# nttcslab-sp/torchain

Measured on AMD Instinct MI355X. Metric: sequence-frames/sec through denominator fwd-bwd, higher is better.
Workload: dtype f32

## Files before the change

### torchain_amd/csrc/chain_internal.h

```cpp
#pragma once

#include <hip/hip_runtime.h>

#include <cstdint>
#include <map>
#include <mutex>
#include <string>
#include <vector>

#include "torchain_hip.h"

namespace tc {

constexpr int kThreads = 1024;
constexpr int kWaves = kThreads / 64;
constexpr int kJvSmall = 2048 / kThreads, kPvSmall = 1024 / kThreads, kJvLarge = 4096 / kThreads, kPvLarge = 3072 / kThreads;
constexpr int kPvMid = 2048 / kThreads;
constexpr int kJvMid = 3072 / kThreads;
constexpr int kMaxRowLen = 32;
constexpr int kLdsLimitBytes = 160 * 1024;

struct ArcRec {
  float w;
  uint32_t idx;
};

constexpr uint32_t kRowFlag = 1u;
constexpr int kStreamUnroll = 16;
constexpr int kStreamUnrollTied = 8;
constexpr int kTiedMinChunks = 6;
constexpr int kMaxIndex = 1 << 14;
constexpr int kJvPlanes = 7;
constexpr int kMaxPlanePositions = 4096 * kJvPlanes;
constexpr int kJvPlanesSplit = 10;
constexpr int kMaxSplitPositions = 4096 * kJvPlanesSplit;

struct ScheduleHost {
  std::vector<ArcRec> cells;
  std::vector<uint32_t> cells6;
  std::vector<int2> wave_range;
  std::vector<int32_t> fix_begin;
  std::vector<int2> fix;
  int32_t extra_slots = 0;
  int64_t conflict_cost = 0, conflict_free_cost = 0, conflict_bound = 0;
  int64_t real_arcs = 0, padded_arcs = 0;
  int32_t rows = 0;
  std::vector<uint32_t> masks;
  int32_t mask_stride = 0;
  std::vector<int32_t> extra_first;
  int32_t nfix = 0;
  int32_t subs = 0;
  int32_t halves = 1;
};

struct ScheduleDev {
  const ArcRec *cells;
  const int2 *wave_range;
  const int32_t *fix_begin;
  const int2 *fix;
  const uint32_t *masks = nullptr;
  const int32_t *extra_first = nullptr;
  int32_t mask_stride = 0, nfix = 0;
  const void *cells_pair = nullptr;
  int32_t subs = 0;
  int32_t halves = 1;
};

constexpr int kSlabRowsPerBlock = 64;
struct SlabRow {
  int32_t row;
  int32_t n;
  int32_t f_off, s_off;
  float ws, pi;
  float K;
  float pad;
};
struct SlabListDev {
  const SlabRow *rows = nullptr;
  const int2 *head = nullptr;
  const uint32_t *rec = nullptr;
  int32_t bundles = 0;
};
struct SlabListHost {
  int W = 2, G = 16;
  std::vector<SlabRow> rows;
  std::vector<int32_t> head;
  std::vector<uint32_t> rec;
  int32_t bundles = 0;
};

struct BigDev {
  SlabListDev in, out, pdf;
  int G = 16;
  int in_blocks = 0, out_blocks = 0;
  int hb = 0;
  int tied = 0;
  const int32_t *f_off = nullptr;
};

struct DenGraphDev {
  BigDev big;
  ScheduleDev fwd, bwd;
  const float *pi;
  const uint32_t *tied_fs = nullptr;
  const float *tied_w = nullptr;
  void *blob = nullptr;
  int pair_choice = -1;
  float tune_ms[2] = {0.f, 0.f};
};

struct DenBestArc {
  int32_t src, pdf;
  float logw;
};
struct DenBestDev {
  const int32_t *in_begin = nullptr;
  const DenBestArc *arcs = nullptr;
  const float *logpi = nullptr;
  void *blob = nullptr;
};
struct DenBestParams {
  DenBestDev t;
  const float *y;
  int64_t y_stride;
  int y_bct, elem;
  int S, T, H, P, Hs;
  const int32_t *seq_frames;
  float *hist;
  int32_t *pdf_out;
  int32_t *state_out;
  double *score_out;
  int resident;
};
constexpr int kDenBestSmallLds = 1024;
inline int64_t den_best_row_floats(int H) { return ((int64_t)H + 3) & ~(int64_t)3; }
inline bool den_best_resident(int H) { return 2 * 4 * den_best_row_floats(H) + kDenBestSmallLds <= (int64_t)160 * 1024; }
inline int64_t den_best_workspace_bytes(int H, int S, int T) {
  return (((int64_t)S * (T + 1) * den_best_row_floats(H) * 4) + 255) & ~(int64_t)255;
}

struct DenLayout {
  int Hs, Ps;
  int off_a, off_acc, off_g, off_al, off_red, off_asum, total_floats;
  bool alpha_in_lds;
  int off_p2;
  int JV, PV;
  int acc_floats;
  bool planewise = false;
  bool asum_global = false;
  int src_planes = 0;
};

struct DenParams {
  ScheduleDev fwd, bwd;
  const float *pi;
  const float *y;
  int64_t y_stride;
  float *deriv;
  int64_t deriv_stride;
  float *alpha_hist;
  float *asum_g = nullptr;
  float *src_scratch = nullptr, *part_scratch = nullptr;
  double *seq_logprob;
  double *seq_y2;
  float *seq_ab;
  float *seq_gsum;
  int S, T, H, P;
  float leaky, deriv_weight, l2_scale;
  int y_vec, d_vec;
  uint32_t seq_frames_lo = 0;
  float *xent_zero = nullptr;
  int64_t xent_stride = 0;
  int x_vec = 0;
  DenLayout L;
  const uint32_t *tied_fs;
  const float *tied_w;
  int gen_owner = 0;
  uint32_t seq_frames_hi = 0;
  BigDev big;
  float *big_expy;
  int64_t big_exp_stride = 0;
  float *big_beta;
  float *big_y;
  uint32_t *big_gam = nullptr;
  float *big_small;
  int big_Sp;
  float big_sum_pi;
  long long *stamps;
  float *beta_hist = nullptr;
  float *fwd_norm = nullptr;
  float *bwd_norm = nullptr;
  float *pair_norm = nullptr;
  uint32_t *pair_sync = nullptr;
  long long *pair_stamps = nullptr;
  int pair_extra_slots = 0;
  int pair_choice = 0;
  uint32_t *mitm_sync = nullptr;
  __host__ __device__ const int32_t *seq_frames() const {
    return reinterpret_cast<const int32_t *>(((uint64_t)seq_frames_hi << 32) | seq_frames_lo);
  }
  void set_seq_frames(const int32_t *f) {
    seq_frames_lo = (uint32_t)(uintptr_t)f;
    seq_frames_hi = (uint32_t)((uint64_t)(uintptr_t)f >> 32);
  }
};

__device__ __forceinline__ int ragged_frames(const int32_t *seq_frames, int s, int T) {
  const int f = __builtin_amdgcn_readfirstlane(seq_frames[s]);
  return f < 1 ? 1 : (f > T ? T : f);
}

}

struct tc_den_graph {
  int32_t H = 0, P = 0;
  int64_t A = 0;
  std::vector<int32_t> arc_src, arc_dst, arc_pdf;
  std::vector<float> arc_prob;
  std::vector<float> initial_probs;
  tc::ScheduleHost fwd, bwd;
  bool tied = false;
  bool gen_owner = false;
  std::vector<uint32_t> tied_fs;
  std::vector<float> tied_w;
  std::vector<uint32_t> tied_fs_state;
  std::vector<float> tied_w_state;
  int32_t work_H = 0;
  std::vector<int32_t> work_src, work_dst, work_pdf, copy_first;
  std::vector<float> work_prob, work_pi;
  std::vector<int32_t> pos;
  std::vector<float> pi_pos;
  tc::DenLayout layout;
  bool layout_ok = false;
  bool big = false;
  tc::SlabListHost big_in, big_out, big_pdf;
  int big_hb = 0;
  int big_G = 16;
  std::vector<int32_t> big_f_off;
  std::vector<int32_t> tied_f, tied_s;
  float big_sum_pi = 0.f;
  std::mutex mu;
  std::map<int, tc::DenGraphDev> dev;
  std::map<int, int> preset_variant;
  std::map<int, tc::DenBestDev> best_dev;
};

namespace tc {

struct NumTables {
  std::vector<int32_t> seq_state_off, seq_arc_off, seq_uniq_off;
  std::vector<int32_t> level_begin;
  std::vector<int32_t> out_begin;
  std::vector<int32_t> in_begin;
  std::vector<int32_t> in_arc;
  std::vector<int32_t> arc_src, arc_dst, arc_uniq;
  std::vector<float> arc_logw;
  std::vector<float> final_logw;
  std::vector<int32_t> uniq_t, uniq_pdf;
  std::vector<int32_t> uniq_begin;
  std::vector<int32_t> uniq_arc;
  int32_t max_states = 0, max_arcs = 0, max_uniq = 0;
  std::vector<int32_t> frame_uniq;
  int32_t max_level_states = 0, max_level_arcs = 0, max_frame_uniq = 0;
  std::vector<int32_t> seq_level_off;
};

inline size_t num_resident_lds_bytes(int32_t max_states, int32_t max_arcs, int32_t max_uniq) {
  return (size_t)((max_states + 1) & ~1) * 16 + (size_t)((max_uniq + 3) & ~3) * 4 + (size_t)((max_arcs + 3) & ~3) * 4;
}
inline size_t num_windowed_lds_bytes(int32_t level_states, int32_t level_arcs, int32_t frame_uniq) {
  return (size_t)((level_states + 1) & ~1) * 32 + (size_t)((frame_uniq + 3) & ~3) * 4 + (size_t)((level_arcs + 3) & ~3) * 4;
}
inline bool num_windowed_fits(size_t dynamic_bytes) { return dynamic_bytes + 2048 <= (size_t)kLdsLimitBytes; }

struct E2eTables {
  std::vector<int32_t> state_off, arc_off, pdf_off, start;
  std::vector<int32_t> in_begin, out_begin;
  std::vector<uint32_t> in_key, out_key;
  std::vector<float> in_lw, out_lw;
  std::vector<int32_t> pdf_begin, pdf_arc;
  std::vector<int32_t> pdf_of;
  std::vector<float> final_lw;
  int32_t max_states = 0, max_arcs = 0, max_pdfs = 0;
  int64_t total_states = 0, total_pdfs = 0;
};

constexpr int64_t kE2eMaxScratchBytes = (int64_t)4 << 30;
struct E2eDev {
  const int32_t *state_off, *arc_off, *pdf_off, *start, *in_begin, *out_begin, *pdf_begin, *pdf_arc, *pdf_of;
  const uint32_t *in_key, *out_key;
  const float *in_lw, *out_lw, *final_lw;
  double *alpha_hist;
  int32_t max_states, max_arcs, max_pdfs;
  int32_t occ_off256;
};
static_assert(sizeof(E2eDev) == 15 * sizeof(void *) + 16, "E2eDev: NumParams' layout is part of the resident kernels' code");

struct PoolSlot {
  char *blob = nullptr, *host = nullptr;
  size_t cap = 0;
  hipEvent_t ready = nullptr, done = nullptr;
};

struct NumDev {
  const int32_t *seq_state_off, *seq_arc_off, *seq_uniq_off, *level_begin, *out_begin, *in_begin, *in_arc,
      *arc_src, *arc_dst, *arc_uniq, *uniq_t, *uniq_pdf, *uniq_begin, *uniq_arc;
  const float *arc_logw, *final_logw;
  const int32_t *frame_uniq = nullptr;
  double *alpha_hist = nullptr;
  float *stage = nullptr;
  PoolSlot *slot = nullptr;
  size_t upload_bytes = 0;
  bool uploaded = false;
  int e2e = 0;
  E2eDev e2e_tab = {};
};

struct NumParams {
  NumDev t;
  const float *y;
  int64_t y_stride;
  float *deriv;
  int64_t deriv_stride;
  float *xent;
  int64_t xent_stride;
  double *seq_logprob;
  int S, T, P;
  float weight;
  float deriv_scale = 1.f, xent_scale = 1.f;
  int staged = 0;
  const float *xent_out = nullptr;
  int64_t xent_out_stride = 0;
  double *seq_xent = nullptr;
  int xent_bct = 0, xent_out_bct = 0, y_bct = 0;
  int lds_states, lds_arcs, lds_uniq;
  int win_states, win_arcs, win_uniq;
  int elem = TC_DTYPE_F32;
  const float *xent_row_w = nullptr;
  const int32_t *seq_frames = nullptr;
  const int32_t *seq_level_off = nullptr;
  int32_t *best_pdf = nullptr;
  double *best_score = nullptr;
  const float *xent_lse = nullptr;
};

}

struct tc_supervision {
  float weight = 1.f;
  int32_t S = 0, T = 0, P = 0;
  bool e2e = false;
  tc::NumTables tab;
  tc::E2eTables e2e_tab;
  std::vector<int32_t> frames;
  int64_t total_frames = 0;
  std::vector<size_t> blob_off;
  std::mutex mu;
  std::map<int, tc::NumDev> dev;
  std::map<int, const int32_t *> frames_dev;
  std::map<int, const int32_t *> level_off_dev;
};

namespace tc {

int build_schedules(tc_den_graph *g);
void build_general(tc_den_graph *g);
bool detect_tied(tc_den_graph *g, std::vector<char> *special);
bool make_work_graph(tc_den_graph *g);
bool build_owner(tc_den_graph *g, const std::vector<char> &special, int max_row, bool count_only = false, bool general = false);
int arrange_half(const std::vector<std::vector<int64_t>> &lane_arcs, int steps, const int32_t *other,
                 const int32_t *pdf, std::vector<std::vector<int>> *pos_out);
int arrange_half_matching(const std::vector<std::vector<int64_t>> &lane_arcs, int steps, const int32_t *other,
                          std::vector<std::vector<int>> *pos_out, std::vector<std::vector<int>> *pad_bank,
                          int *lower_bound);
inline int round4(int x) { return (x + 3) & ~3; }
bool compute_layout(int H, int P, int T_hint, int extra_slots, bool tied, DenLayout *L, bool need_alpha = false);
constexpr int asum_stride(int T) { return (T + 2 + 3) & ~3; }
bool compute_layout_planes(int Npos, int P, int T_hint, int extra_slots, DenLayout *L);
int64_t layout_lds_bytes(const DenLayout &L, int T);

hipError_t allow_dynamic_lds(const void *kernel, size_t lds_bytes);
int launch_den(const DenParams &p, hipStream_t stream);
int launch_den_big(const DenParams &p, int accumulate, hipStream_t stream);
int launch_den_tied(const DenParams &p, int accumulate, hipStream_t stream);
int launch_den_general_owner(const DenParams &p, int accumulate, hipStream_t stream);
int launch_den_tied_planes(const DenParams &p, int accumulate, hipStream_t stream);
bool planes_mitm_fits(const DenParams &p);
int launch_den_tied_planes_mitm(const DenParams &p, int accumulate, hipStream_t stream);
int launch_den_tied_backward_only(const DenParams &p, hipStream_t stream);
int launch_den_tied_combine(const DenParams &p, int accumulate, int num_cus, hipStream_t stream);
bool split_bwd_fits(const DenLayout &L, int T);
constexpr int kSplitMaxSeq = 128;
int launch_den_tied_pair(const DenParams &p, int extra_slots, int accumulate, hipStream_t stream);
bool pair_fits(const DenLayout &L, int extra_slots, int T);
int tune_den_variant(tc_den_graph *g, int device);
std::string tuning_cache_key(uint64_t graph_hash, const char *device_name);
bool tuning_cache_get(const std::string &key, int *two_sequence_kernel);
void tuning_cache_put(const std::string &key, int two_sequence_kernel, float fused_ms, float two_sequence_ms);
int launch_den_tied_mitm(const DenParams &p, uint32_t *sync, int accumulate, hipStream_t stream);
bool mitm_fits(const DenLayout &L, int T);
size_t mitm_sync_bytes(int S);
int pair_norm_stride(int T);
size_t pair_sync_bytes(int S);
inline size_t pair_stamp_bytes(int T) { return ((size_t)2 * kWaves * (T + 2) * 8 * 8 + 255) & ~(size_t)255; }
int64_t big_small_floats(int hb, int P, int T, int Sp);
int launch_num(const NumParams &p, hipStream_t stream);
int launch_num_scatter(const NumParams &p, hipStream_t stream);
int launch_num_windowed(const NumParams &p, hipStream_t stream);
int launch_num_e2e(const NumParams &p, hipStream_t stream);
int launch_num_e2e_scatter(const NumParams &p, hipStream_t stream);
int launch_num_best_path(const NumParams &p, hipStream_t stream);
int launch_den_best_path(const DenBestParams &p, hipStream_t stream);
int den_best_tables(tc_den_graph *g, int device, DenBestDev *out);
inline size_t num_e2e_lds_bytes(int max_states, int max_arcs, int max_pdfs) {
  return (size_t)2 * ((max_states + 3) & ~3) * sizeof(double) + (((max_pdfs + 3) & ~3) + (size_t)max_arcs) * sizeof(float);
}
int launch_num_e2e_large(const NumParams &p, hipStream_t stream);
inline bool e2e_beyond_resident(int max_states, int max_arcs, int max_pdfs) {
  return max_states > TC_E2E_MAX_STATES || max_arcs > TC_E2E_MAX_ARCS || max_pdfs > TC_E2E_MAX_PDFS;
}
inline bool e2e_large_fits(int states, int pdfs) {
  return num_windowed_fits((size_t)16 * ((states + 3) & ~3) + (size_t)4 * ((pdfs + 3) & ~3));
}
inline size_t e2e_seq_lds_bytes(int max_states, int max_pdfs) {
  const size_t both = num_e2e_lds_bytes(max_states, 0, max_pdfs), rule = (size_t)kLdsLimitBytes - 2048;
  return both < rule ? both : rule;
}
struct SideStreams {
  hipStream_t den_side = nullptr, num_side = nullptr;
  hipEvent_t fork = nullptr, join = nullptr, num_fork = nullptr, num_join = nullptr;
  int num_cus = 0;
  std::recursive_mutex enqueue;
};
int side_streams(hipStream_t stream, SideStreams **out);
void side_streams_forget(hipStream_t stream);
int den_cus_used(const DenParams &p, int num_cus);
bool den_zeroes_xent(const DenParams &p, int num_cus);
int launch_finalize(const double *den_lp, const double *num_lp, const double *y2, const float *ab, const float *gs,
                    int S, int T, float sup_weight, float l2, int have_deriv, float *results, int32_t *fail_flag,
                    hipStream_t stream, const double *xent_lp = nullptr, double *xent_total = nullptr,
                    float *loss_out = nullptr, int64_t total_frames = 0);
int launch_finalize_per_sequence(const double *den_lp, const double *num_lp, const double *y2, const float *ab, const float *gs,
                                 int S, int T, float sup_weight, float l2, int have_deriv, float *results, int32_t *fail_flag,
                                 hipStream_t stream, const double *xent_lp, double *xent_total, float *loss_out,
                                 int64_t total_frames, const int32_t *seq_frames, int isolate, double *seq_results,
                                 int32_t *alive_frames);
int launch_zero_failed(void *out, int elem_bytes, int64_t sb, int64_t st, int64_t sc, int B, int T, int cols,
                       const int32_t *alive_frames, hipStream_t stream);
int launch_zero_padding(void *out, int elem_bytes, int64_t sb, int64_t st, int64_t sc, int B, int T, int cols,
                        const int32_t *seq_frames, hipStream_t stream);
int launch_zero_on_fail(const int32_t *fail_flag, float *a, int64_t a_stride, float *b, int64_t b_stride,
                        const float *y, int64_t y_stride, float l2_scale, int64_t rows, int cols, hipStream_t stream);
int launch_den_reduce(const double *den_lp, const float *ab, const float *gs, int S, double *logprob_out,
                      int32_t *status_out, hipStream_t stream);
int launch_sum_double(const double *in, int n, double scale, double *out, hipStream_t stream);
int launch_xent_total(const double *in, int n, const int32_t *fail_flag, double *out, hipStream_t stream);
int launch_step_loss(const float *results3, float *loss1, hipStream_t stream);
int64_t trace_workspace_bytes();
int launch_trace_mat_mat(const float *a, int64_t a_stride, const float *b, int64_t b_stride, int64_t rows, int cols,
                         double *partial, double *out, hipStream_t stream);
constexpr float kOutputLimit = 30.0f;
struct LastPass {
  float scale = 1.0f;
  const float *row_w = nullptr;
  float pen_c2 = 0.0f;
  const void *y = nullptr;
  int64_t y_stride = 0, y_st = 0;
  bool scaled = true;
};
bool layout_grid_ok(int B, int T);
int launch_to2d(int dtype, const void *in_bct, float *out, int B, int Cn, int T, int64_t stride2d, hipStream_t stream);
int launch_from2d(int dtype, const float *in, int64_t stride2d, void *out_bct, int B, int Cn, int T, const LastPass &lp,
                  hipStream_t stream);
int launch_widen_rows(int dtype, const void *in, int64_t in_stride, float *out, int64_t rows, int cols, hipStream_t stream);
int launch_round(int dtype, const float *in, void *out, int64_t n, int cols, const LastPass &lp, hipStream_t stream);
int launch_scale_rows(float *a, int64_t rows, int cols, const LastPass &lp, hipStream_t stream);
bool channel_last_strides_ok(int B, int T, int cols, int64_t sb, int64_t st);
int launch_rows_gather(int dtype, const void *x, int64_t sb, int64_t st, float *out, int64_t out_stride, int B, int T, int cols,
                       hipStream_t stream);
int launch_rows_scatter(int dtype, const float *in, int64_t in_stride, void *out, int64_t osb, int64_t ost, int B, int T,
                        int cols, const LastPass &lp, hipStream_t stream);

int launch_xent_row_stats(int dtype, const void *x, int x_bct, int64_t x_stride, int S, int T, int P, float *stats,
                          hipStream_t stream);
int launch_xent_softmax_grad(int dtype, const void *x, int x_bct, int64_t x_stride, float *g, int64_t g_stride, int S, int T,
                             int P, const float *stats, const int32_t *live_frames, hipStream_t stream);

extern thread_local int g_last_hip_error;

constexpr int kKernelGeneration = 6;
enum DebugFlag { kDbgForceGeneral = 0, kDbgForceStreamed, kDbgNoSplit, kDbgNoPdfBanks, kDbgNoBankSearch, kDbgSchedTrace, kDbgNoPhaseSplit, kDbgNoNumOverlap, kDbgNoPair, kDbgForcePair, kDbgNoTune, kDbgNoMitm, kDbgForceMitm, kDbgSlabWide, kDbgSlabNarrow, kDbgExpPerFrame, kDbgOldArrange, kDbgNoPlanes, kDbgOldGeneral, kDbgPhantomPdf0, kDbgNoPdfSearch, kDbgNoSplitSrc, kDbgPlanesMeetAt, kDbgForceNumWindowed, kDbgForceDenBestStreamed, kDbgForceNumE2eLarge, kDbgCount };
bool debug_flag(DebugFlag f);
int debug_value(DebugFlag f);

int pool_acquire(int device, size_t bytes, PoolSlot **out);
void pool_release(int device, PoolSlot *slot);
int64_t pool_counter(int which);
enum LaunchCounter { kCntDen = 0, kCntDenBackward, kCntNum, kCntNumBackward, kCntLayout, kCntDenAsumGlobal, kCntNumE2eStaged, kCntNumWindowed, kCntChannelLast, kCntRagged, kCntRaggedTwoCu, kCntBestPath, kCntDenBestPath, kCntDenBestPathStreamed, kCntXentLogSoftmax, kCntNumE2eLarge, kCntCount };
void count_launch(LaunchCounter c);
int supervision_mark_use(tc_supervision *sup, int device, hipStream_t stream);
int stage_e2e_locked(tc_supervision *sup, int device);
int supervision_from_example(const tc_example *ex, tc_supervision **out);
#define TC_HIP_CHECK(expr)                        \
  do {                                            \
    hipError_t e__ = (expr);                      \
    if (e__ != hipSuccess) {                      \
      tc::g_last_hip_error = (int)e__;            \
      return TC_ERR_HIP;                          \
    }                                             \
  } while (0)

}
```

### torchain_amd/csrc/den_graph.cpp

```cpp
#include <algorithm>
#include <atomic>
#include <array>
#include <cctype>
#include <cmath>
#include <cstdio>
#include <cstring>
#include <numeric>
#include <string>

#include "chain_internal.h"

namespace tc {

thread_local int g_last_hip_error = 0;

hipError_t allow_dynamic_lds(const void *kernel, size_t lds_bytes) {
  static std::mutex mu;
  static std::map<std::pair<const void *, int>, size_t> granted;
  int device = 0;
  hipError_t e = hipGetDevice(&device);
  if (e != hipSuccess) return e;
  std::lock_guard<std::mutex> lock(mu);
  size_t &have = granted[std::make_pair(kernel, device)];
  if (have >= lds_bytes) return hipSuccess;
  e = hipFuncSetAttribute(kernel, hipFuncAttributeMaxDynamicSharedMemorySize, (int)lds_bytes);
  if (e == hipSuccess) have = lds_bytes;
  return e;
}

static std::mutex &g_side_mu = *new std::mutex();
static std::map<std::pair<int, hipStream_t>, SideStreams> &g_side_ctx = *new std::map<std::pair<int, hipStream_t>, SideStreams>();

void side_streams_forget(hipStream_t stream) {
  int device = 0;
  if (hipGetDevice(&device) != hipSuccess) return;
  std::lock_guard<std::mutex> lock(g_side_mu);
  auto it = g_side_ctx.find(std::make_pair(device, stream));
  if (it == g_side_ctx.end()) return;
  SideStreams &c = it->second;
  for (hipStream_t x : {c.den_side, c.num_side})
    if (x) {
      (void)hipStreamSynchronize(x);
      (void)hipStreamDestroy(x);
    }
  for (hipEvent_t x : {c.fork, c.join, c.num_fork, c.num_join})
    if (x) (void)hipEventDestroy(x);
  g_side_ctx.erase(it);
}

int side_streams(hipStream_t stream, SideStreams **out) {
  std::mutex &mu = g_side_mu;
  auto &ctx = g_side_ctx;
  int device = 0;
  TC_HIP_CHECK(hipGetDevice(&device));
  std::lock_guard<std::mutex> lock(mu);
  SideStreams &c = ctx[std::make_pair(device, stream)];
  if (!c.den_side) {
    int num_cus = 0;
    TC_HIP_CHECK(hipDeviceGetAttribute(&num_cus, hipDeviceAttributeMultiprocessorCount, device));
    hipEvent_t ev[4] = {nullptr, nullptr, nullptr, nullptr};
    hipStream_t st[2] = {nullptr, nullptr};
    hipError_t e = hipSuccess;
    for (int i = 0; i < 4 && e == hipSuccess; ++i) e = hipEventCreateWithFlags(&ev[i], hipEventDisableTiming);
    for (int i = 0; i < 2 && e == hipSuccess; ++i) e = hipStreamCreateWithFlags(&st[i], hipStreamNonBlocking);
    if (e != hipSuccess) {
      for (hipEvent_t x : ev)
        if (x) (void)hipEventDestroy(x);
      for (hipStream_t x : st)
        if (x) (void)hipStreamDestroy(x);
      g_last_hip_error = (int)e;
      return TC_ERR_HIP;
    }
    c.fork = ev[0];
    c.join = ev[1];
    c.num_fork = ev[2];
    c.num_join = ev[3];
    c.num_side = st[0];
    c.den_side = st[1];
    c.num_cus = num_cus;
  }
  *out = &c;
  return TC_OK;
}

static std::atomic<int> g_debug[kDbgCount];
bool debug_flag(DebugFlag f) { return g_debug[f].load(std::memory_order_relaxed) != 0; }
int debug_value(DebugFlag f) { return g_debug[f].load(std::memory_order_relaxed); }
static std::atomic<int64_t> g_launches[kCntCount];
void count_launch(LaunchCounter c) { g_launches[c].fetch_add(1, std::memory_order_relaxed); }

struct SlabEntry {
  uint32_t d[4];
};
static uint32_t f2u(float f) {
  uint32_t u;
  std::memcpy(&u, &f, 4);
  return u;
}

static void make_slab_list(int W, int G, const std::vector<std::vector<SlabEntry>> &entries, const std::vector<SlabRow> &meta,
                           const std::vector<int32_t> &bundle_rows, SlabListHost *out) {
  const int spc = 16 / W, NG = 64 / G, CH = NG * 16;
  out->W = W;
  out->G = G;
  out->bundles = (int32_t)(bundle_rows.size() / NG);
  out->rows.assign(bundle_rows.size(), SlabRow{-1, 0, -1, -1, 0.f, 0.f, 0.f, 0.f});
  out->head.assign((size_t)out->bundles * 2, 0);
  out->rec.clear();
  size_t chunk = 0;
  for (int32_t b = 0; b < out->bundles; ++b) {
    const int32_t *br = &bundle_rows[(size_t)b * NG];
    const bool shared = NG > 1 && br[1] == -2;
    int steps = 0;
    if (shared) {
      steps = ((int)entries[br[0]].size() + NG - 1) / NG;
    } else {
      for (int q = 0; q < NG; ++q)
        if (br[q] >= 0) steps = std::max(steps, (int)entries[br[q]].size());
    }
    const int chunks = (steps + spc - 1) / spc;
    out->head[(size_t)b * 2] = (int32_t)chunk;
    out->head[(size_t)b * 2 + 1] = shared ? (int32_t)((uint32_t)steps | 0x80000000u) : steps;
    out->rec.resize((chunk + chunks) * CH, 0u);
    auto put = [&](int q, int i, const SlabEntry &e) {
      for (int c = 0; c < W; ++c) out->rec[(chunk + i / spc) * CH + q * 16 + (i % spc) * W + c] = e.d[c];
    };
    if (shared) {
      const int32_t r = br[0];
      const int n = (int)entries[r].size();
      for (int q = 0; q < NG; ++q) {
        SlabRow m = q == 0 ? meta[r] : SlabRow{-1, 0, -1, -1, 0.f, 0.f, 0.f, 0.f};
        m.n = (n - q + NG - 1) / NG;
        out->rows[(size_t)b * NG + q] = m;
      }
      for (int i = 0; i < n; ++i) put(i % NG, i / NG, entries[r][i]);
    } else {
      for (int q = 0; q < NG; ++q) {
        const int32_t r = br[q];
        if (r < 0) continue;
        SlabRow m = meta[r];
        m.n = (int32_t)entries[r].size();
        out->rows[(size_t)b * NG + q] = m;
        for (int i = 0; i < m.n; ++i) put(q, i, entries[r][i]);
      }
    }
    chunk += chunks;
  }
  out->rec.resize((chunk + 3) * CH, 0u);
}

constexpr size_t kSlabHubLen = 48;
static std::vector<int32_t> bundles_by_length(const std::vector<std::vector<SlabEntry>> &entries, int G) {
  const int NG = 64 / G;
  std::vector<int32_t> order(entries.size());
  std::iota(order.begin(), order.end(), 0);
  std::stable_sort(order.begin(), order.end(), [&](int32_t a, int32_t b) { return entries[a].size() > entries[b].size(); });
  std::vector<int32_t> out;
  size_t i = 0;
  for (; NG > 1 && i < order.size() && entries[order[i]].size() >= kSlabHubLen; ++i) {
    out.push_back(order[i]);
    for (int q = 1; q < NG; ++q) out.push_back(-2);
  }
  for (; i < order.size(); ++i) out.push_back(order[i]);
  while (out.size() % NG) out.push_back(-1);
  if (out.empty()) out.assign(NG, -1);
  return out;
}

static std::vector<int32_t> bundles_by_tile(const std::vector<std::vector<SlabEntry>> &entries, int P) {
  std::vector<int32_t> out;
  for (int p0 = 0; p0 < P; p0 += 64) {
    std::vector<int32_t> tile(64, -1);
    for (int i = 0; i < 64 && p0 + i < P; ++i) tile[i] = p0 + i;
    std::stable_sort(tile.begin(), tile.end(), [&](int32_t a, int32_t b) {
      const size_t na = a >= 0 ? entries[a].size() + 1 : 0, nb = b >= 0 ? entries[b].size() + 1 : 0;
      return na > nb;
    });
    out.insert(out.end(), tile.begin(), tile.end());
  }
  return out;
}

static void build_big(tc_den_graph *g) {
  const int H = g->H, P = g->P, G = g->big_G;
  const uint32_t rb = 4u * G;
  const int64_t A = g->A;
  std::vector<std::vector<SlabEntry>> in(H), outl(H), pdf(P);
  for (int64_t a = 0; a < A; ++a) {
    const uint32_t s = (uint32_t)g->arc_src[a] * rb, d = (uint32_t)g->arc_dst[a] * rb, pd = (uint32_t)g->arc_pdf[a] * rb;
    const uint32_t w = f2u(g->arc_prob[a]), pis = f2u(g->initial_probs[g->arc_src[a]]);
    in[g->arc_dst[a]].push_back(SlabEntry{{s, pd, w, pis}});
    outl[g->arc_src[a]].push_back(SlabEntry{{d, pd, w, f2u(1.0f)}});
    pdf[g->arc_pdf[a]].push_back(SlabEntry{{s, d, w, pis}});
  }
  std::vector<SlabRow> ms(H), mp(P);
  for (int h = 0; h < H; ++h) ms[h] = SlabRow{h, 0, -1, -1, 0.f, g->initial_probs[h], 0.f, 0.f};
  for (int i = 0; i < P; ++i) mp[i] = SlabRow{i, 0, -1, -1, 0.f, 0.f, 0.f, 0.f};
  make_slab_list(4, G, in, ms, bundles_by_length(in, G), &g->big_in);
  make_slab_list(4, G, outl, ms, bundles_by_length(outl, G), &g->big_out);
  make_slab_list(4, G, pdf, mp, bundles_by_tile(pdf, P), &g->big_pdf);
  g->big_f_off.assign(1, -1);
  float sum_pi = 0.f;
  for (int h = 0; h < H; ++h) sum_pi += g->initial_probs[h];
  g->big_sum_pi = sum_pi;
}

static void build_big_tied(tc_den_graph *g, const std::vector<char> &special) {
  const int H = g->work_H, G = g->big_G;
  const uint32_t rb = 4u * G;
  const int64_t A = (int64_t)g->work_src.size();
  std::vector<std::vector<SlabEntry>> in(H), outl(H);
  std::vector<float> K(H, 0.f);
  for (int64_t a = 0; a < A; ++a) {
    if (special[a]) continue;
    const int32_t s = g->work_src[a], d = g->work_dst[a];
    in[d].push_back(SlabEntry{{(uint32_t)s * rb, f2u(g->work_prob[a]), 0u, 0u}});
    outl[s].push_back(SlabEntry{{(uint32_t)d * rb, f2u(g->work_prob[a]), 0u, 0u}});
    K[d] += g->work_prob[a] * g->work_pi[s];
  }
  std::vector<SlabRow> mi(H), mo(H);
  g->big_f_off.assign(H, -1);
  for (int h = 0; h < H; ++h) {
    const int32_t f = g->tied_f[h] >= 0 ? g->tied_f[h] * (int32_t)rb : -1, sl = g->tied_s[h] >= 0 ? g->tied_s[h] * (int32_t)rb : -1;
    mi[h] = SlabRow{h, 0, f, sl, g->tied_w[h], g->work_pi[h], K[h], 0.f};
    mo[h] = SlabRow{h, 0, f, sl, g->tied_w[h], g->work_pi[h], 0.f, 0.f};
    g->big_f_off[h] = f;
  }
  make_slab_list(2, G, in, mi, bundles_by_length(in, G), &g->big_in);
  make_slab_list(2, G, outl, mo, bundles_by_length(outl, G), &g->big_out);
  g->big_pdf = SlabListHost();
  float sum_pi = 0.f;
  for (int h = 0; h < H; ++h) sum_pi += g->work_pi[h];
  g->big_sum_pi = sum_pi;
}

int build_schedules(tc_den_graph *g) {
  bool want_big = debug_flag(kDbgForceStreamed) || g->H > kMaxSplitPositions || g->P > kMaxIndex;
  bool split_made = false;
  std::vector<char> special;
  {
    g->work_H = g->H;
    g->work_src = g->arc_src;
    g->work_dst = g->arc_dst;
    g->work_pdf = g->arc_pdf;
    g->work_prob = g->arc_prob;
    g->work_pi = g->initial_probs;
    g->copy_first.resize(g->H + 1);
    std::iota(g->copy_first.begin(), g->copy_first.end(), 0);
    bool tied = !debug_flag(kDbgForceGeneral) && detect_tied(g, &special);
    if (!tied && !debug_flag(kDbgForceGeneral) && !debug_flag(kDbgNoSplit) && make_work_graph(g)) {
      tied = detect_tied(g, &special);
      split_made = tied;
    }
    g->tied = tied;
    if (!tied && g->H > kMaxIndex) want_big = true;
  }
  auto restore_unsplit = [&]() {
    g->work_H = g->H;
    g->work_src = g->arc_src;
    g->work_dst = g->arc_dst;
    g->work_pdf = g->arc_pdf;
    g->work_prob = g->arc_prob;
    g->work_pi = g->initial_probs;
    g->copy_first.resize(g->H + 1);
    std::iota(g->copy_first.begin(), g->copy_first.end(), 0);
    g->tied = false;
    g->gen_owner = false;
    g->tied_fs.clear();
    g->tied_w.clear();
    g->fwd = ScheduleHost();
    g->bwd = ScheduleHost();
  };
  auto general_owner = [&]() {
    if (debug_flag(kDbgOldGeneral)) return false;
    const std::vector<char> none(g->work_src.size(), 0);
    int fit_row = 0;
    int64_t best_cells = -1;
    for (int max_row = kMaxRowLen; max_row <= 8 * kMaxRowLen; max_row *= 2) {
      if (!build_owner(g, none, max_row, true, true)) continue;
      const int64_t cells = g->fwd.padded_arcs + g->bwd.padded_arcs;
      if (best_cells < 0 || cells < best_cells) {
        best_cells = cells;
        fit_row = max_row;
      }
    }
    if (!fit_row || !build_owner(g, none, fit_row, false, true)) {
      g->fwd = ScheduleHost();
      g->bwd = ScheduleHost();
      return false;
    }
    g->gen_owner = true;
    g->layout_ok = true;
    return true;
  };
  if (!want_big && g->tied) {
    int fit_row = 0;
    {
      int64_t best_cells = -1;
      for (int max_row = kMaxRowLen; max_row <= 8 * kMaxRowLen; max_row *= 2) {
        if (!build_owner(g, special, max_row, true)) continue;
        const int64_t cells = g->fwd.padded_arcs + g->bwd.padded_arcs;
        if (best_cells < 0 || cells < best_cells) {
          best_cells = cells;
          fit_row = max_row;
        }
        if (debug_flag(kDbgSchedTrace)) fprintf(stderr, "[sched] rows cut at %d: %lld cells, %d bytes of LDS\n", max_row, (long long)cells, 4 * g->layout.total_floats);
      }
      if (fit_row && !build_owner(g, special, fit_row)) {
        fit_row = 0;
        for (int max_row = kMaxRowLen; max_row <= 8 * kMaxRowLen && !fit_row; max_row *= 2)
          if (build_owner(g, special, max_row)) fit_row = max_row;
      }
    }
    if (fit_row) {
      g->layout_ok = true;
      return TC_OK;
    }
    if (split_made && g->H <= kMaxIndex) {
      std::vector<char> special_split = special;
      std::vector<int32_t> ws = g->work_src, wd = g->work_dst, wp = g->work_pdf, cf = g->copy_first, tf = g->tied_f, ts = g->tied_s;
      std::vector<float> wpr = g->work_prob, wpi = g->work_pi, tw = g->tied_w;
      std::vector<uint32_t> tfs = g->tied_fs;
      const int32_t wH = g->work_H;
      restore_unsplit();
      if (general_owner()) return TC_OK;
      build_general(g);
      g->layout_ok = compute_layout(g->H, g->P, 256, std::max(g->fwd.extra_slots, g->bwd.extra_slots), false, &g->layout);
      if (g->layout_ok) return TC_OK;
      g->work_H = wH;
      g->work_src.swap(ws);
      g->work_dst.swap(wd);
      g->work_pdf.swap(wp);
      g->work_prob.swap(wpr);
      g->work_pi.swap(wpi);
      g->copy_first.swap(cf);
      g->tied_f.swap(tf);
      g->tied_s.swap(ts);
      g->tied_w.swap(tw);
      g->tied_fs.swap(tfs);
      g->tied = true;
      special.swap(special_split);
    }
    want_big = true;
  }
  if (!want_big) {
    if (g->work_H != g->H) restore_unsplit();
    if (general_owner()) return TC_OK;
    build_general(g);
    g->layout_ok = compute_layout(g->H, g->P, 256, std::max(g->fwd.extra_slots, g->bwd.extra_slots), false, &g->layout);
    if (g->layout_ok) return TC_OK;
  }
  g->big = true;
  {
    const int64_t states = g->tied ? g->work_H : g->H;
    g->big_G = states >= 28000 ? 32 : 16;
    if (debug_flag(kDbgSlabWide)) g->big_G = 32;
    if (debug_flag(kDbgSlabNarrow)) g->big_G = 16;
  }
  g->layout_ok = false;
  g->fwd = ScheduleHost();
  g->bwd = ScheduleHost();
  if (g->tied)
    build_big_tied(g, special);
  else
    build_big(g);
  g->big_hb = (std::max(g->big_in.bundles, g->big_out.bundles) + g->big_G - 1) / g->big_G;
  return TC_OK;
}

}

using namespace tc;

extern "C" {

int tc_debug_set(const char *key, int value) {
  static const char *const names[kDbgCount] = {"force_general", "force_streamed", "no_split", "no_pdf_banks",
                                               "no_bank_search", "sched_trace", "no_phase_split", "no_num_overlap", "no_pair",
                                               "force_pair", "no_tune", "no_mitm", "force_mitm", "slab_wide", "slab_narrow", "exp_per_frame", "old_arrange", "no_planes", "old_general", "phantom_pdf0", "no_pdf_search", "no_split_source", "planes_meet_at", "force_num_windowed", "force_den_best_path_streamed", "force_num_e2e_large"};
  if (!key) return TC_ERR_INVALID_ARGUMENT;
  for (int i = 0; i < kDbgCount; ++i)
    if (!strcmp(key, names[i])) {
      g_debug[i].store(value, std::memory_order_relaxed);
      return TC_OK;
    }
  return TC_ERR_INVALID_ARGUMENT;
}

namespace {
const bool g_env_applied = [] {
  const char *env = getenv("TORCHAIN_HIP_DEBUG");
  if (!env) return false;
  std::string all(env);
  size_t pos = 0;
  while (pos <= all.size()) {
    size_t end = all.find(',', pos);
    if (end == std::string::npos) end = all.size();
    std::string item = all.substr(pos, end - pos);
    pos = end + 1;
    if (item.empty()) continue;
    int value = 1;
    const size_t eq = item.find('=');
    if (eq != std::string::npos) {
      value = atoi(item.c_str() + eq + 1);
      item.resize(eq);
    }
    if (tc_debug_set(item.c_str(), value) != TC_OK) fprintf(stderr, "libtorchain_hip: unknown switch '%s' in TORCHAIN_HIP_DEBUG\n", item.c_str());
  }
  return true;
}();
}

int64_t tc_debug_counter(const char *key) {
  if (key && !strcmp(key, "pool_device_allocs")) return pool_counter(0);
  if (key && !strcmp(key, "pool_reuses")) return pool_counter(1);
  static const char *const names[kCntCount] = {"den_launches", "den_backward_launches", "num_launches", "num_backward_launches", "layout_launches",
                                              "den_long_utterance_launches", "num_e2e_staged_launches", "num_windowed_launches", "channel_last_steps", "ragged_steps", "ragged_two_cu_launches", "best_path_launches", "den_best_path_launches", "den_best_path_streamed_launches", "xent_log_softmax_launches", "num_e2e_large_launches"};
  for (int i = 0; key && i < kCntCount; ++i)
    if (!strcmp(key, names[i])) return g_launches[i].load(std::memory_order_relaxed);
  return -1;
}

int tc_den_graph_create(tc_den_graph **out, int32_t num_states, int64_t num_arcs, const int32_t *arc_src,
                        const int32_t *arc_dst, const int32_t *arc_ilabel, const float *arc_weight,
                        const float *final_weight, int32_t start_state, int32_t num_pdfs) {
  if (!out) return TC_ERR_INVALID_ARGUMENT;
  *out = nullptr;
  if (num_states <= 0 || num_arcs < 0 || num_pdfs <= 0 || !final_weight) return TC_ERR_INVALID_ARGUMENT;
  if (num_arcs > 0 && (!arc_src || !arc_dst || !arc_ilabel || !arc_weight)) return TC_ERR_INVALID_ARGUMENT;
  if (start_state < 0 || start_state >= num_states) return TC_ERR_BAD_FST;
  if (num_arcs >= (int64_t)1 << 30) return TC_ERR_UNSUPPORTED;
  for (int64_t a = 0; a < num_arcs; ++a) {
    if (arc_src[a] < 0 || arc_src[a] >= num_states || arc_dst[a] < 0 || arc_dst[a] >= num_states)
      return TC_ERR_BAD_FST;
    if (arc_ilabel[a] < 1 || arc_ilabel[a] > num_pdfs) return TC_ERR_BAD_FST;
    if (a > 0 && arc_src[a] < arc_src[a - 1]) return TC_ERR_BAD_FST;
    if (!(arc_weight[a] == arc_weight[a])) return TC_ERR_BAD_FST;
  }
  tc_den_graph *g = new tc_den_graph();
  g->H = num_states;
  g->P = num_pdfs;
  g->A = num_arcs;
  g->arc_src.assign(arc_src, arc_src + num_arcs);
  g->arc_dst.assign(arc_dst, arc_dst + num_arcs);
  g->arc_pdf.resize(num_arcs);
  g->arc_prob.resize(num_arcs);
  for (int64_t a = 0; a < num_arcs; ++a) {
    g->arc_pdf[a] = arc_ilabel[a] - 1;
    g->arc_prob[a] = (float)std::exp(-(double)arc_weight[a]);
  }
  {
    const int H = num_states;
    std::vector<double> norm(H), cur(H, 0.0), nxt(H, 0.0), avg(H, 0.0);
    for (int s = 0; s < H; ++s) norm[s] = std::exp(-(double)final_weight[s]);
    for (int64_t a = 0; a < num_arcs; ++a) norm[arc_src[a]] += std::exp(-(double)arc_weight[a]);
    for (int s = 0; s < H; ++s)
      if (!(norm[s] > 0.0) || !std::isfinite(norm[s])) {
        delete g;
        return TC_ERR_BAD_FST;
      }
    for (int s = 0; s < H; ++s) norm[s] = 1.0 / norm[s];
    cur[start_state] = 1.0;
    for (int iter = 0; iter < 100; ++iter) {
      for (int s = 0; s < H; ++s) avg[s] += cur[s] * (1.0 / 100);
      for (int64_t a = 0; a < num_arcs; ++a) {
        int s = arc_src[a];
        nxt[arc_dst[a]] += cur[s] * norm[s] * std::exp(-(double)arc_weight[a]);
      }
      double sum = 0.0;
      for (int s = 0; s < H; ++s) sum += nxt[s];
      for (int s = 0; s < H; ++s) {
        cur[s] = nxt[s] * (1.0 / sum);
        nxt[s] = 0.0;
      }
    }
    g->initial_probs.resize(H);
    for (int s = 0; s < H; ++s) g->initial_probs[s] = (float)avg[s];
  }
  build_schedules(g);
  *out = g;
  return TC_OK;
}

}

namespace {
struct Reader {
  FILE *f;
  bool ok = true;
  template <class T>
  T get() {
    T v{};
    if (fread(&v, sizeof(T), 1, f) != 1) ok = false;
    return v;
  }
  std::string str() {
    int32_t n = get<int32_t>();
    if (!ok || n < 0 || n > (1 << 20)) {
      ok = false;
      return std::string();
    }
    std::string s((size_t)n, '\0');
    if (n && fread(&s[0], 1, (size_t)n, f) != (size_t)n) ok = false;
    return s;
  }
  void skip_symbol_table() {
    int32_t magic = get<int32_t>();
    if (magic != 2125658996) {
      ok = false;
      return;
    }
    str();
    get<int64_t>();
    int64_t size = get<int64_t>();
    for (int64_t i = 0; ok && i < size; ++i) {
      str();
      get<int64_t>();
    }
  }
};
}

extern "C" {

int tc_den_graph_read(tc_den_graph **out, const char *rxfilename, int32_t num_pdfs) {
  if (!out || !rxfilename) return TC_ERR_INVALID_ARGUMENT;
  *out = nullptr;
  std::string name(rxfilename);
  while (!name.empty() && isspace((unsigned char)name.back())) name.pop_back();
  const bool is_pipe = !name.empty() && name.back() == '|';
  if (is_pipe) name.pop_back();
  FILE *f = is_pipe ? popen(name.c_str(), "r") : fopen(name.c_str(), "rb");
  if (!f) return TC_ERR_IO;
  Reader r{f};
  int rc = TC_OK;
  std::vector<int32_t> src, dst, il;
  std::vector<float> w, fin;
  int64_t start = 0, nstates = 0;
  try {
  do {
    if (r.get<int32_t>() != 2125659606) { rc = TC_ERR_IO; break; }
    std::string fsttype = r.str(), arctype = r.str();
    int32_t version = r.get<int32_t>(), flags = r.get<int32_t>();
    r.get<uint64_t>();
    start = r.get<int64_t>();
    nstates = r.get<int64_t>();
    int64_t narcs = r.get<int64_t>();
    if (!r.ok || fsttype != "vector" || arctype != "standard" || version < 2 || (flags & 4)  ||
        nstates <= 0 || nstates > (1 << 24)) {
      rc = TC_ERR_IO;
      break;
    }
    if (flags & 1) r.skip_symbol_table();
    if (flags & 2) r.skip_symbol_table();
    if (narcs > 0 && narcs <= (1 << 24)) { src.reserve(narcs); dst.reserve(narcs); il.reserve(narcs); w.reserve(narcs); }
    fin.resize(nstates);
    for (int64_t s = 0; r.ok && s < nstates; ++s) {
      fin[s] = r.get<float>();
      int64_t n = r.get<int64_t>();
      if (!r.ok || n < 0 || n > (1 << 28)) { r.ok = false; break; }
      for (int64_t i = 0; r.ok && i < n; ++i) {
        int32_t ilabel = r.get<int32_t>();
        r.get<int32_t>();
        float weight = r.get<float>();
        int32_t next = r.get<int32_t>();
        src.push_back((int32_t)s);
        dst.push_back(next);
        il.push_back(ilabel);
        w.push_back(weight);
      }
    }
    if (!r.ok) rc = TC_ERR_IO;
  } while (0);
  } catch (...) {
    rc = TC_ERR_IO;
  }
  if (is_pipe) {
    if (pclose(f) != 0 && rc == TC_OK) rc = TC_ERR_IO;
  } else {
    fclose(f);
  }
  if (rc != TC_OK) return rc;
  return tc_den_graph_create(out, (int32_t)nstates, (int64_t)src.size(), src.data(), dst.data(), il.data(), w.data(),
                             fin.data(), (int32_t)start, num_pdfs);
}

void tc_den_graph_free(tc_den_graph *g) {
  if (!g) return;
  for (auto &kv : g->dev) {
    if (kv.second.blob) {
      int cur = 0;
      if (hipGetDevice(&cur) == hipSuccess) {
        (void)hipSetDevice(kv.first);
        (void)hipFree(kv.second.blob);
        (void)hipSetDevice(cur);
      }
    }
  }
  for (auto &kv : g->best_dev) {
    int cur = 0;
    if (kv.second.blob && hipGetDevice(&cur) == hipSuccess) {
      (void)hipSetDevice(kv.first);
      (void)hipFree(kv.second.blob);
      (void)hipSetDevice(cur);
    }
  }
  delete g;
}

int32_t tc_den_graph_num_states(const tc_den_graph *g) { return g ? g->H : 0; }
int64_t tc_den_graph_num_arcs(const tc_den_graph *g) { return g ? g->A : 0; }
int32_t tc_den_graph_num_pdfs(const tc_den_graph *g) { return g ? g->P : 0; }

int tc_den_graph_initial_probs(const tc_den_graph *g, float *out_host) {
  if (!g || !out_host) return TC_ERR_INVALID_ARGUMENT;
  memcpy(out_host, g->initial_probs.data(), sizeof(float) * (size_t)g->H);
  return TC_OK;
}

int tc_den_graph_stats(const tc_den_graph *g, int64_t *o) {
  if (!g || !o) return TC_ERR_INVALID_ARGUMENT;
  o[0] = g->fwd.padded_arcs;
  o[1] = g->bwd.padded_arcs;
  o[2] = g->layout_ok ? layout_lds_bytes(g->layout, 150) : -1;
  o[3] = kThreads;
  o[4] = g->fwd.rows;
  o[5] = g->bwd.rows;
  o[6] = g->fwd.conflict_free_cost ? 1000 * g->fwd.conflict_cost / g->fwd.conflict_free_cost : 0;
  o[7] = g->bwd.conflict_free_cost ? 1000 * g->bwd.conflict_cost / g->bwd.conflict_free_cost : 0;
  o[8] = g->big ? 2 : (g->tied ? 1 : 0);
  return TC_OK;
}

int tc_den_graph_debug_walk(const tc_den_graph *g, int direction, const float *gather, const float *pdf_factor,
                            float *out) {
  if (!g || !gather || !pdf_factor || !out || direction < 0 || direction > 1) return TC_ERR_INVALID_ARGUMENT;
  const int H = g->H;
  auto slab_sums = [&](const SlabListHost &L, auto term, std::vector<float> *sums) {
    const int spc = 16 / L.W, NG = 64 / L.G, CH = NG * 16;
    for (int32_t b = 0; b < L.bundles; ++b) {
      const bool shared = L.head[(size_t)b * 2 + 1] < 0;
      float gsum[4] = {0.f, 0.f, 0.f, 0.f};
      for (int q = 0; q < NG; ++q) {
        const SlabRow &r = L.rows[(size_t)b * NG + q];
        if (r.row < 0 && !shared) continue;
        float sum = 0.f;
        for (int i = 0; i < r.n; ++i) sum += term(&L.rec[((size_t)L.head[(size_t)b * 2] + i / spc) * CH + q * 16 + (i % spc) * L.W]);
        if (shared)
          gsum[q] = sum;
        else
          (*sums)[r.row] = sum;
      }
      if (shared) (*sums)[L.rows[(size_t)b * NG].row] = NG == 4 ? (gsum[0] + gsum[1]) + (gsum[2] + gsum[3]) : gsum[0] + gsum[1];
    }
  };
  auto u2f = [](uint32_t u) {
    float f;
    std::memcpy(&f, &u, 4);
    return f;
  };
  if (g->big && g->tied) {
    const SlabListHost &L = direction == 0 ? g->big_in : g->big_out;
    auto pf = [&](int pdf) { return pdf >= 0 ? pdf_factor[pdf] : 0.f; };
    std::vector<float> val(g->work_H, 0.f), sums(g->work_H, 0.f);
    for (int h = 0; h < H; ++h)
      for (int c = g->copy_first[h]; c < g->copy_first[h + 1]; ++c)
        val[c] = direction == 0 ? (c == g->copy_first[h] ? gather[h] : 0.f) : gather[h] * pf(g->tied_f[c]);
    slab_sums(L, [&](const uint32_t *e) { return u2f(e[1]) * val[e[0] / (4 * L.G)]; }, &sums);
    for (int h = 0; h < H; ++h) {
      float total = 0.f;
      for (int c = g->copy_first[h]; c < g->copy_first[h + 1]; ++c) {
        const float own = direction == 0 ? (c == g->copy_first[h] ? gather[h] : 0.f) : gather[h];
        const float self = pf(g->tied_s[c]) * g->tied_w[c] * own;
        const float v = direction == 0 ? pf(g->tied_f[c]) * sums[c] + self : sums[c] + self;
        if (direction == 1) {
          total = v;
          break;
        }
        total += v;
      }
      out[h] = total;
    }
    return TC_OK;
  }
  if (g->big) {
    std::vector<float> sums(H, 0.f);
    slab_sums(direction == 0 ? g->big_in : g->big_out,
              [&](const uint32_t *e) { return u2f(e[2]) * gather[e[0] / (4 * g->big_G)] * pdf_factor[e[1] / (4 * g->big_G)]; }, &sums);
    for (int h = 0; h < H; ++h) out[h] = sums[h];
    return TC_OK;
  }
  if (!g->layout_ok) return TC_ERR_UNSUPPORTED;
  const ScheduleHost &sc = direction == 0 ? g->fwd : g->bwd;
  const int Hs = g->layout.Hs;
  std::vector<float> acc((size_t)std::max(g->layout.acc_floats, Hs + 4 + sc.extra_slots) + 64, 0.f);
  if (g->gen_owner) {
    const int K = Hs / kThreads;
    std::vector<float> src_pos((size_t)Hs + 4, 0.f);
    for (int h = 0; h < H; ++h) src_pos[g->pos[h]] = gather[h];
    for (int w = 0; w < kWaves; ++w) {
      const int first = sc.wave_range[w].x, n = sc.wave_range[w].y;
      for (int l = 0; l < 64; ++l) {
        const int tid = 64 * w + l;
        int k = 0;
        float a = 0.f;
        auto slot = [&]() { return k < K ? 4 * (tid + kThreads * (k >> 2)) + (k & 3) : Hs + 4 + 64 * (sc.extra_first[w] + (k - K)) + l; };
        for (int i = 0; i < n; ++i) {
          const size_t c = (size_t)first + i, chunk = c / 8, q = c % 8;
          const uint32_t *base = &sc.cells6[chunk * 4 * 64 * 4];
          const uint32_t x = base[((q / 4) * 64 + l) * 4 + (q % 4)], idx = base[((2 + q / 4) * 64 + l) * 4 + (q % 4)];
          float wgt;
          memcpy(&wgt, &x, 4);
          a += wgt * src_pos[(idx & 0xffffu) >> 2] * pdf_factor[idx >> 18];
          const uint32_t m = sc.masks[(size_t)w * sc.mask_stride + (i / 2) / 8];
          const int bit = (i / 2) % 8;
          if ((m >> ((i & 1) ? bit : 8 + bit)) & 1u) {
            acc[slot()] = a;
            ++k;
            a = 0.f;
          }
        }
      }
    }
    for (size_t t = 0; t + 1 < sc.fix_begin.size(); ++t)
      for (int e = sc.fix_begin[t]; e < sc.fix_begin[t + 1]; ++e) acc[sc.fix[e].x] += acc[sc.fix[e].y];
    for (int h = 0; h < H; ++h) out[h] = acc[g->pos[h]];
    return TC_OK;
  }
  if (g->tied) {
    const int K = Hs / kThreads;
    const bool pw = g->layout.planewise;
    const int subs = pw ? sc.subs : 1, halves = pw ? sc.halves : 1, subs_all = subs * halves;
    const int half_pos = halves == 2 ? 4096 * ((Hs / 4096 + 1) / 2) : 0;
    std::vector<float> total(acc.size(), 0.f);
    std::vector<float> src_pos((size_t)Hs + 4, 0.f);
    for (int h = 0; h < H; ++h)
      for (int c = g->copy_first[h]; c < g->copy_first[h + 1]; ++c) {
        const uint32_t fs = g->tied_fs[g->pos[c]];
        src_pos[g->pos[c]] = direction == 0 ? (c == g->copy_first[h] ? gather[h] : 0.f)
                                            : gather[h] * pdf_factor[(fs & 0xffffu) >> 2];
      }
    for (int hv = 0; hv < halves; ++hv) {
    std::fill(acc.begin(), acc.end(), 0.f);
    const int pos_base = hv ? half_pos : 0;
    for (int w = 0; w < kWaves; ++w)
     for (int sub = 0; sub < subs; ++sub) {
      const int first = sc.wave_range[(size_t)w * subs_all + hv * subs + sub].x;
      const int rel = pw ? first - sc.wave_range[(size_t)w * subs_all].x : 0;
      const int n = sc.wave_range[(size_t)w * subs_all + hv * subs + sub].y - rel;
      for (int l = 0; l < 64; ++l) {
        const int tid = 64 * w + l;
        int k = !pw ? 0 : sub == 0 ? K : 4 * (sub - 1);
        float ax = 0.f, ay = 0.f;
        auto slot = [&]() {
          return k < K ? 4 * (tid + kThreads * (k >> 2)) + (k & 3) : Hs + 4 + 64 * (sc.extra_first[w] + (k - K)) + l;
        };
        auto cell = [&](int i, float *wgt, int *position) {
          const size_t c = (size_t)first + i, chunk = c / 8, q = c % 8;
          const uint32_t *base = &sc.cells6[chunk * 3 * 64 * 4];
          uint32_t x = base[((q / 4) * 64 + l) * 4 + (q % 4)];
          memcpy(wgt, &x, 4);
          const uint32_t o = base[(2 * 64 + l) * 4 + q / 2];
          *position = pos_base + (int)(((q & 1) ? o >> 16 : o & 0xffffu) >> (pw ? 0 : 2));
        };
        for (int i = 0; i < n; i += 2) {
          float w0, w1;
          int p0, p1;
          cell(i, &w0, &p0);
          cell(i + 1, &w1, &p1);
          uint32_t m = pw ? 0u : sc.masks[((size_t)w * subs + sub) * sc.mask_stride + (i / 2) / 8];
          int bit = (i / 2) % 8;
          if (pw) {
            const int cell = rel + i, chunk = cell / 8;
            const uint32_t byte = (sc.masks[(size_t)w * sc.mask_stride + chunk / 4] >> (8 * (chunk % 4))) & 0xffu;
            m = (((byte >> (cell % 8)) & 1u) << 8) | ((byte >> (cell % 8 + 1)) & 1u);
            bit = 0;
          }
          if ((m >> (8 + bit)) & 1u) {
            acc[slot()] = (ax + w0 * src_pos[p0]) + ay;
            ++k;
            ax = 0.f;
            ay = w1 * src_pos[p1];
          } else {
            ax += w0 * src_pos[p0];
            ay += w1 * src_pos[p1];
          }
          if ((m >> bit) & 1u) {
            acc[slot()] = ax + ay;
            ++k;
            ax = ay = 0.f;
          }
        }
      }
    }
    const size_t lists = (sc.fix_begin.size() - 1) / (size_t)halves;
    for (size_t t = hv * lists; t < (hv + 1) * lists; ++t)
      for (int e = sc.fix_begin[t]; e < sc.fix_begin[t + 1]; ++e) {
        const size_t tl = t - hv * lists;
        if (pw && ((sc.fix[e].x >> 2) % kThreads != (int)(tl / (K / 4)) || sc.fix[e].x / (4 * kThreads) != (int)(tl % (K / 4))))
          return TC_ERR_UNSUPPORTED;
        acc[sc.fix[e].x] += acc[sc.fix[e].y];
      }
    for (int p = 0; p < Hs; ++p) total[p] += acc[p];
    }
    acc.swap(total);
    for (int h = 0; h < H; ++h) {
      float sum = 0.f;
      for (int c = g->copy_first[h]; c < g->copy_first[h + 1]; ++c) {
        const int p = g->pos[c];
        const uint32_t fs = g->tied_fs[p];
        const float self = pdf_factor[fs >> 18] * g->tied_w[p] * (direction == 0 && c != g->copy_first[h] ? 0.f : gather[h]);
        const float v = direction == 0 ? pdf_factor[(fs & 0xffffu) >> 2] * acc[p] + self : acc[p] + self;
        if (direction == 1) {
          sum = v;
          break;
        }
        sum += v;
      }
      out[h] = sum;
    }
    return TC_OK;
  }
  for (int w = 0; w < kWaves; ++w) {
    const int first = sc.wave_range[w].x, n = sc.wave_range[w].y;
    for (int l = 0; l < 64; ++l) {
      int cur = Hs;
      float a = 0.f;
      for (int i = 0; i < n; ++i) {
        const size_t c = (size_t)first + i;
        const ArcRec &r = sc.cells[((c >> 1) * 64 + l) * 2 + (c & 1)];
        if (r.idx & kRowFlag) {
          acc[cur] = a;
          uint32_t x;
          memcpy(&x, &r.w, 4);
          cur = (int)(x & 0xffffu);
          a = 0.f;
        } else {
          a += r.w * gather[std::min<uint32_t>(r.idx >> 18, (uint32_t)H - 1)] * pdf_factor[(r.idx >> 2) & 0x3fffu];
        }
      }
    }
  }
  for (int t = 0; t < kThreads; ++t)
    for (int e = sc.fix_begin[t]; e < sc.fix_begin[t + 1]; ++e) acc[sc.fix[e].x] += acc[sc.fix[e].y];
  for (int h = 0; h < H; ++h) out[h] = acc[h];
  return TC_OK;
}

static int upload_den_graph(tc_den_graph *g, int device);

int tc_den_graph_prepare(tc_den_graph *g, int device) {
  if (!g) return TC_ERR_INVALID_ARGUMENT;
  const int rc = upload_den_graph(g, device);
  if (rc != TC_OK) return rc;
  return tune_den_variant(g, device);
}

static int upload_den_graph(tc_den_graph *g, int device) {
  std::lock_guard<std::mutex> lock(g->mu);
  if (g->dev.count(device)) return TC_OK;
  int prev = 0;
  TC_HIP_CHECK(hipGetDevice(&prev));
  TC_HIP_CHECK(hipSetDevice(device));
  const int Hs = (g->H + 3) & ~3;
  auto align = [](size_t x) { return (x + 255) & ~(size_t)255; };
  struct Part { const void *src; size_t bytes; size_t off; };
  if (g->big) {
    const std::vector<float> &pi_src = g->tied ? g->work_pi : g->initial_probs;
    std::vector<float> pi_pad(pi_src.size() + 8, 0.f);
    std::copy(pi_src.begin(), pi_src.end(), pi_pad.begin());
    const std::vector<int32_t> none_i(1, -1);
    const std::vector<float> none_f(1, 0.f);
    const bool tb = g->tied;
    const SlabListHost *lists[3] = {&g->big_in, &g->big_out, &g->big_pdf};
    const std::vector<SlabRow> no_rows(4, SlabRow{-1, 0, -1, -1, 0.f, 0.f, 0.f, 0.f});
    const std::vector<int32_t> no_head(2, 0);
    const std::vector<uint32_t> no_rec(256, 0u);
    Part parts[11];
    for (int l = 0; l < 3; ++l) {
      const bool have = lists[l]->bundles > 0;
      parts[3 * l] = Part{have ? (const void *)lists[l]->rows.data() : no_rows.data(), (have ? lists[l]->rows.size() : 4) * sizeof(SlabRow), 0};
      parts[3 * l + 1] = Part{have ? (const void *)lists[l]->head.data() : no_head.data(), (have ? lists[l]->head.size() : 2) * 4, 0};
      parts[3 * l + 2] = Part{have ? (const void *)lists[l]->rec.data() : no_rec.data(), (have ? lists[l]->rec.size() : 256) * 4, 0};
    }
    parts[9] = Part{pi_pad.data(), pi_pad.size() * 4, 0};
    parts[10] = Part{g->big_f_off.data(), g->big_f_off.size() * 4, 0};
    size_t total = 0;
    for (auto &p : parts) {
      p.off = total;
      total += align(p.bytes);
    }
    char *blob = nullptr;
    hipError_t e = hipMalloc((void **)&blob, total);
    if (e == hipSuccess)
      for (auto &p : parts) {
        e = hipMemcpy(blob + p.off, p.src, p.bytes, hipMemcpyHostToDevice);
        if (e != hipSuccess) break;
      }
    (void)hipSetDevice(prev);
    if (e != hipSuccess) {
      g_last_hip_error = (int)e;
      return TC_ERR_HIP;
    }
    DenGraphDev d;
    d.blob = blob;
    SlabListDev *dl[3] = {&d.big.in, &d.big.out, &d.big.pdf};
    for (int l = 0; l < 3; ++l) {
      dl[l]->rows = (const SlabRow *)(blob + parts[3 * l].off);
      dl[l]->head = (const int2 *)(blob + parts[3 * l + 1].off);
      dl[l]->rec = (const uint32_t *)(blob + parts[3 * l + 2].off);
      dl[l]->bundles = lists[l]->bundles;
    }
    d.pi = (const float *)(blob + parts[9].off);
    d.big.tied = tb ? 1 : 0;
    d.big.G = g->big_G;
    d.big.in_blocks = (g->big_in.bundles + g->big_G - 1) / g->big_G;
    d.big.out_blocks = (g->big_out.bundles + g->big_G - 1) / g->big_G;
    d.big.hb = g->big_hb;
    d.big.f_off = (const int32_t *)(blob + parts[10].off);
    g->dev[device] = d;
    return TC_OK;
  }
  std::vector<float> pi_pad(Hs + 4, 0.f);
  std::copy(g->initial_probs.begin(), g->initial_probs.end(), pi_pad.begin());
  if (g->tied || g->gen_owner) pi_pad = g->pi_pos;
  const std::vector<uint32_t> no_mask(1, 0u);
  const std::vector<int32_t> no_extra(kWaves, 0);
  std::vector<uint32_t> pair_cells[2];
  const bool want_pair = g->tied && g->layout.Hs <= 8192 && !g->fwd.cells6.empty();
  if (want_pair)
    for (int dir = 0; dir < 2; ++dir) {
      const std::vector<uint32_t> &src = dir == 0 ? g->fwd.cells6 : g->bwd.cells6;
      pair_cells[dir] = src;
      for (size_t chunk = 0; chunk + 1 <= src.size() / (3 * 64 * 4); ++chunk)
        for (size_t i = 0; i < 64 * 4; ++i) {
          uint32_t &x = pair_cells[dir][chunk * 3 * 64 * 4 + 2 * 64 * 4 + i];
          x = ((x & 0xffffu) << 1) | ((x >> 16) << 17);
        }
    }
  const std::vector<uint32_t> no_pair(4, 0u);
  Part parts[] = {
      {g->fwd.cells6.empty() ? (const void *)g->fwd.cells.data() : (const void *)g->fwd.cells6.data(),
       g->fwd.cells6.empty() ? g->fwd.cells.size() * sizeof(ArcRec) : g->fwd.cells6.size() * 4, 0},
      {g->fwd.wave_range.data(), g->fwd.wave_range.size() * sizeof(int2), 0},
      {g->bwd.cells6.empty() ? (const void *)g->bwd.cells.data() : (const void *)g->bwd.cells6.data(),
       g->bwd.cells6.empty() ? g->bwd.cells.size() * sizeof(ArcRec) : g->bwd.cells6.size() * 4, 0},
      {g->bwd.wave_range.data(), g->bwd.wave_range.size() * sizeof(int2), 0},
      {pi_pad.data(), pi_pad.size() * 4, 0},
      {g->fwd.fix_begin.data(), g->fwd.fix_begin.size() * 4, 0},
      {g->fwd.fix.data(), g->fwd.fix.size() * sizeof(int2), 0},
      {g->bwd.fix_begin.data(), g->bwd.fix_begin.size() * 4, 0},
      {g->bwd.fix.data(), g->bwd.fix.size() * sizeof(int2), 0},
      {g->tied_fs.data(), g->tied_fs.size() * 4, 0},
      {g->tied_w.data(), g->tied_w.size() * 4, 0},
      {g->fwd.masks.empty() ? no_mask.data() : g->fwd.masks.data(), std::max<size_t>(1, g->fwd.masks.size()) * 4, 0},
      {g->bwd.masks.empty() ? no_mask.data() : g->bwd.masks.data(), std::max<size_t>(1, g->bwd.masks.size()) * 4, 0},
      {g->fwd.extra_first.empty() ? no_extra.data() : g->fwd.extra_first.data(), kWaves * 4, 0},
      {g->bwd.extra_first.empty() ? no_extra.data() : g->bwd.extra_first.data(), kWaves * 4, 0},
      {want_pair ? pair_cells[0].data() : no_pair.data(), (want_pair ? pair_cells[0].size() : no_pair.size()) * 4, 0},
      {want_pair ? pair_cells[1].data() : no_pair.data(), (want_pair ? pair_cells[1].size() : no_pair.size()) * 4, 0},
  };
  size_t total = 0;
  for (auto &p : parts) {
    p.off = total;
    total += align(p.bytes);
  }
  char *blob = nullptr;
  hipError_t e = hipMalloc((void **)&blob, total);
  if (e == hipSuccess) {
    for (auto &p : parts) {
      e = hipMemcpy(blob + p.off, p.src, p.bytes, hipMemcpyHostToDevice);
      if (e != hipSuccess) break;
    }
  }
  (void)hipSetDevice(prev);
  if (e != hipSuccess) {
    g_last_hip_error = (int)e;
    return TC_ERR_HIP;
  }
  DenGraphDev d;
  d.blob = blob;
  d.fwd = ScheduleDev{(const ArcRec *)(blob + parts[0].off), (const int2 *)(blob + parts[1].off),
                      (const int32_t *)(blob + parts[5].off), (const int2 *)(blob + parts[6].off),
                      (const uint32_t *)(blob + parts[11].off), (const int32_t *)(blob + parts[13].off),
                      g->fwd.mask_stride, g->fwd.nfix};
  d.bwd = ScheduleDev{(const ArcRec *)(blob + parts[2].off), (const int2 *)(blob + parts[3].off),
                      (const int32_t *)(blob + parts[7].off), (const int2 *)(blob + parts[8].off),
                      (const uint32_t *)(blob + parts[12].off), (const int32_t *)(blob + parts[14].off),
                      g->bwd.mask_stride, g->bwd.nfix};
  d.fwd.subs = g->fwd.subs;
  d.bwd.subs = g->bwd.subs;
  d.fwd.halves = g->fwd.halves;
  d.bwd.halves = g->bwd.halves;
  d.pi = (const float *)(blob + parts[4].off);
  if (g->tied) {
    d.tied_fs = (const uint32_t *)(blob + parts[9].off);
    d.tied_w = (const float *)(blob + parts[10].off);
  }
  if (want_pair) {
    d.fwd.cells_pair = blob + parts[15].off;
    d.bwd.cells_pair = blob + parts[16].off;
  }
  g->dev[device] = d;
  return TC_OK;
}

}

int tc::den_best_tables(tc_den_graph *g, int device, DenBestDev *out) {
  std::lock_guard<std::mutex> lock(g->mu);
  auto it = g->best_dev.find(device);
  if (it != g->best_dev.end()) {
    *out = it->second;
    return TC_OK;
  }
  const int H = g->H;
  const int64_t A = g->A;
  std::vector<int32_t> in_begin(H + 1, 0);
  for (int64_t a = 0; a < A; ++a) ++in_begin[g->arc_dst[a] + 1];
  for (int h = 0; h < H; ++h) in_begin[h + 1] += in_begin[h];
  std::vector<DenBestArc> arcs((size_t)std::max<int64_t>(A, 1), DenBestArc{0, 0, -INFINITY});
  {
    std::vector<int32_t> fill(in_begin.begin(), in_begin.end() - 1);
    for (int64_t a = 0; a < A; ++a)
      arcs[fill[g->arc_dst[a]]++] = DenBestArc{g->arc_src[a], g->arc_pdf[a], (float)std::log((double)g->arc_prob[a])};
  }
  std::vector<float> logpi(H);
  for (int h = 0; h < H; ++h) logpi[h] = g->initial_probs[h] > 0.f ? (float)std::log((double)g->initial_probs[h]) : -INFINITY;
  auto align = [](size_t x) { return (x + 255) & ~(size_t)255; };
  const size_t off_arcs = align(in_begin.size() * 4), off_pi = off_arcs + align(arcs.size() * sizeof(DenBestArc));
  const size_t total = off_pi + align(logpi.size() * 4);
  int prev = 0;
  TC_HIP_CHECK(hipGetDevice(&prev));
  TC_HIP_CHECK(hipSetDevice(device));
  char *blob = nullptr;
  hipError_t e = hipMalloc((void **)&blob, total);
  if (e == hipSuccess) e = hipMemcpy(blob, in_begin.data(), in_begin.size() * 4, hipMemcpyHostToDevice);
  if (e == hipSuccess) e = hipMemcpy(blob + off_arcs, arcs.data(), arcs.size() * sizeof(DenBestArc), hipMemcpyHostToDevice);
  if (e == hipSuccess) e = hipMemcpy(blob + off_pi, logpi.data(), logpi.size() * 4, hipMemcpyHostToDevice);
  (void)hipSetDevice(prev);
  if (e != hipSuccess) {
    if (blob) (void)hipFree(blob);
    g_last_hip_error = (int)e;
    return TC_ERR_HIP;
  }
  DenBestDev d;
  d.in_begin = (const int32_t *)blob;
  d.arcs = (const DenBestArc *)(blob + off_arcs);
  d.logpi = (const float *)(blob + off_pi);
  d.blob = blob;
  g->best_dev[device] = d;
  *out = d;
  return TC_OK;
}

extern "C" {

const char *tc_strerror(int code) {
  switch (code) {
    case TC_OK: return "ok";
    case TC_ERR_INVALID_ARGUMENT: return "invalid argument";
    case TC_ERR_BAD_FST: return "malformed FST";
    case TC_ERR_UNSUPPORTED: return "problem size not supported by the on-chip layout";
    case TC_ERR_WORKSPACE: return "workspace missing or too small";
    case TC_ERR_HIP: return "HIP runtime error";
    case TC_ERR_IO: return "cannot read OpenFst vector/standard file";
    case TC_ERR_NOT_SEPARABLE: return "merged supervision FST does not factor per sequence";
    default: return "unknown error";
  }
}

int tc_version(void) { return 100; }
int tc_last_hip_error(void) { return tc::g_last_hip_error; }

}
```

### torchain_amd/csrc/den_tied_device.h

```cpp
#pragma once

#include "den_device.h"

namespace tc {

namespace {

typedef float f4 __attribute__((ext_vector_type(4)));
typedef uint32_t u4 __attribute__((ext_vector_type(4)));
typedef __attribute__((address_space(3))) float lds_f;
typedef __attribute__((address_space(3))) uint32_t lds_u;
typedef __attribute__((address_space(3))) f4 lds_f4;
typedef __attribute__((address_space(3))) u4 lds_u4;

__device__ __forceinline__ float ldsf(uint32_t a) { return *reinterpret_cast<lds_f *>(a); }
__device__ __forceinline__ void ldsf_st(uint32_t a, float v) { *reinterpret_cast<lds_f *>(a) = v; }
__device__ __forceinline__ f4 lds4(uint32_t a) { return *reinterpret_cast<lds_f4 *>(a); }
__device__ __forceinline__ void lds4_st(uint32_t a, f4 v) { *reinterpret_cast<lds_f4 *>(a) = v; }
__device__ __forceinline__ void lds4_st_at(uint32_t base, uint32_t off, f4 v) {
  asm volatile("ds_write_b128 %0, %1 offset:%2" : : "v"(base), "v"(v), "i"(off) : "memory");
}
__device__ __forceinline__ u4 lds4u(uint32_t a) { return *reinterpret_cast<lds_u4 *>(a); }
__device__ __forceinline__ void lds_add_u32(uint32_t a, uint32_t v) {
  __hip_atomic_fetch_add(reinterpret_cast<lds_u *>(a), v, __ATOMIC_RELAXED, __HIP_MEMORY_SCOPE_WORKGROUP);
}

typedef __amdgpu_buffer_rsrc_t rsrc_t;
__device__ __forceinline__ rsrc_t make_rsrc(const void *ubase, uint32_t bytes) {
  return __builtin_amdgcn_make_buffer_rsrc(const_cast<void *>(ubase), 0, (int)bytes, 0x00020000);
}
__device__ __forceinline__ u4 bld4u(rsrc_t r, uint32_t voff, uint32_t soff) {
  return __builtin_amdgcn_raw_buffer_load_b128(r, (int)voff, (int)soff, 0);
}
__device__ __forceinline__ f4 bld4(rsrc_t r, uint32_t voff, uint32_t soff) {
  const u4 v = bld4u(r, voff, soff);
  return f4{__uint_as_float(v.x), __uint_as_float(v.y), __uint_as_float(v.z), __uint_as_float(v.w)};
}
template <int AUX>
__device__ __forceinline__ f4 bld4_aux(rsrc_t r, uint32_t voff, uint32_t soff) {
  const u4 v = __builtin_amdgcn_raw_buffer_load_b128(r, (int)voff, (int)soff, AUX);
  return f4{__uint_as_float(v.x), __uint_as_float(v.y), __uint_as_float(v.z), __uint_as_float(v.w)};
}
__device__ __forceinline__ void bst4(rsrc_t r, uint32_t voff, f4 v) {
#ifndef TC_STORE_AUX
#define TC_STORE_AUX 2
#endif
  __builtin_amdgcn_raw_buffer_store_b128(u4{__float_as_uint(v.x), __float_as_uint(v.y), __float_as_uint(v.z), __float_as_uint(v.w)},
                                         r, (int)voff, 0, TC_STORE_AUX);
}

template <int AUX>
__device__ __forceinline__ void bst4_aux(rsrc_t r, uint32_t voff, f4 v) {
  __builtin_amdgcn_raw_buffer_store_b128(u4{__float_as_uint(v.x), __float_as_uint(v.y), __float_as_uint(v.z), __float_as_uint(v.w)},
                                         r, (int)voff, 0, AUX);
}

__device__ __forceinline__ void dma4_to_lds(rsrc_t r, uint32_t voff, uint32_t lds_wave) {
  uint32_t keep;
  asm volatile("s_mov_b32 %0, m0\n\ts_mov_b32 m0, %3\n\ts_nop 4\n\tbuffer_load_dwordx4 %1, %2, 0 offen lds\n\ts_mov_b32 m0, %0"
               : "=&s"(keep)
               : "v"(voff), "s"(r), "s"(lds_wave)
               : "memory");
}
template <int N>
__device__ __forceinline__ void dma_wait() {
  static_assert(N >= 0 && N < 64, "vmcnt is a 6-bit count");
  asm volatile("s_waitcnt vmcnt(%0)" : : "n"(N) : "memory");
}
__device__ __forceinline__ void lds_wait_all() { asm volatile("s_waitcnt lgkmcnt(0)" : : : "memory"); }

__device__ __forceinline__ f4 mk4(float x) { return f4{x, x, x, x}; }
__device__ __forceinline__ float hsum(f4 v) { return (v.x + v.y) + (v.z + v.w); }
__device__ __forceinline__ float exp_med3(float x) { return __expf(__builtin_amdgcn_fmed3f(x, -30.0f, 30.0f)); }
__device__ __forceinline__ f4 exp4(f4 y) { return f4{exp_med3(y.x), exp_med3(y.y), exp_med3(y.z), exp_med3(y.w)}; }

__device__ __forceinline__ f4 row_ld(rsrc_t r, uint32_t voff, int vec) {
  if (vec) return bld4(r, voff, 0);
  return f4{__uint_as_float(__builtin_amdgcn_raw_buffer_load_b32(r, (int)voff, 0, 0)),
            __uint_as_float(__builtin_amdgcn_raw_buffer_load_b32(r, (int)voff, 4, 0)),
            __uint_as_float(__builtin_amdgcn_raw_buffer_load_b32(r, (int)voff, 8, 0)),
            __uint_as_float(__builtin_amdgcn_raw_buffer_load_b32(r, (int)voff, 12, 0))};
}
__device__ __forceinline__ void row_st(rsrc_t r, uint32_t voff, int vec, f4 v) {
  if (vec) {
    bst4(r, voff, v);
  } else {
    __builtin_amdgcn_raw_buffer_store_b32(__float_as_uint(v.x), r, (int)voff, 0, 0);
    __builtin_amdgcn_raw_buffer_store_b32(__float_as_uint(v.y), r, (int)voff, 4, 0);
    __builtin_amdgcn_raw_buffer_store_b32(__float_as_uint(v.z), r, (int)voff, 8, 0);
    __builtin_amdgcn_raw_buffer_store_b32(__float_as_uint(v.w), r, (int)voff, 12, 0);
  }
}

__device__ __forceinline__ float block_sum_a(float v, uint32_t red, int wave, uint32_t lane) {
  v = wave_sum(v);
  if (lane == 0) ldsf_st(red + 4u * (uint32_t)wave, v);
  __syncthreads();
  static_assert(kWaves == 16, "one DPP row holds the wave totals");
  float t = ldsf(red + 4u * (lane & 15u));
  t = dpp_add<0xB1>(t);
  t = dpp_add<0x4E>(t);
  t = dpp_add<0x124>(t);
  t = dpp_add<0x128>(t);
  return t;
}

__device__ __forceinline__ void gamma_add_a(uint32_t addr, float v) {
  int32_t q;
  asm("v_cvt_rpi_i32_f32 %0, %1" : "=v"(q) : "v"(v));
  lds_add_u32(addr, (uint32_t)q);
}

struct Chunk6 {
  u4 wa, wb, oc;
};

__device__ __forceinline__ void load_chunk(Chunk6 &q, rsrc_t stream, uint32_t lane16, int chunk) {
  const uint32_t so = (uint32_t)chunk * (3 * 64 * 16);
  q.wa = bld4u(stream, lane16, so);
  q.wb = bld4u(stream, lane16, so + 1024);
  q.oc = bld4u(stream, lane16, so + 2048);
}

__device__ __forceinline__ uint32_t lo16(uint32_t x) {
  uint32_t r;
  asm volatile("v_and_b32 %0, 0xffff, %1" : "=v"(r) : "v"(x));
  return r;
}
__device__ __forceinline__ uint32_t hi16(uint32_t x) {
  uint32_t r;
  asm volatile("v_lshrrev_b32 %0, 16, %1" : "=v"(r) : "v"(x));
  return r;
}

__device__ __forceinline__ uint32_t lo16w(uint32_t x) {
  uint32_t r;
  const uint32_t two = 2u;
  asm volatile("v_lshlrev_b32_sdwa %0, %1, %2 dst_sel:DWORD dst_unused:UNUSED_PAD src0_sel:DWORD src1_sel:WORD_0" : "=v"(r) : "s"(two), "v"(x));
  return r;
}
__device__ __forceinline__ uint32_t hi16w(uint32_t x) {
  uint32_t r;
  const uint32_t two = 2u;
  asm volatile("v_lshlrev_b32_sdwa %0, %1, %2 dst_sel:DWORD dst_unused:UNUSED_PAD src0_sel:DWORD src1_sel:WORD_1" : "=v"(r) : "s"(two), "v"(x));
  return r;
}

struct RowCommit {
  uint32_t row;
  uint32_t sec_row;
  int left;
  __device__ __forceinline__ void commit(float v) {
    asm volatile("s_mov_b32 m0, %1\n\ts_nop 0\n\tds_write_addtid_b32 %0" : : "v"(v), "s"(row) : "memory", "m0");
    --left;
    row = left == 0 ? sec_row : row + 256u;
  }
};

template <uint32_t SRC, int HALF>
__device__ __forceinline__ void do_chunk(const Chunk6 &q, uint32_t m, float &acc, RowCommit &rc) {
  uint32_t o[8];
  o[0] = lo16(q.oc.x);
  o[1] = hi16(q.oc.x);
  o[2] = lo16(q.oc.y);
  o[3] = hi16(q.oc.y);
  o[4] = lo16(q.oc.z);
  o[5] = hi16(q.oc.z);
  o[6] = lo16(q.oc.w);
  o[7] = hi16(q.oc.w);
  float a[8];
#pragma unroll
  for (int i = 0; i < 8; ++i) {
#ifdef TC_ABL_NOGATHER
    a[i] = __uint_as_float(o[i]);
#else
    a[i] = ldsf(SRC + o[i]);
#endif
  }
  const uint32_t w[8] = {q.wa.x, q.wa.y, q.wa.z, q.wa.w, q.wb.x, q.wb.y, q.wb.z, q.wb.w};
#pragma unroll
  for (int i = 0; i < 8; ++i) {
    acc = fmaf(a[i], __uint_as_float(w[i]), acc);
    const int bit = (i & 1) ? 4 * HALF + i / 2 : 8 + 4 * HALF + i / 2;
    if (__builtin_expect((m >> bit) & 1u, 0)) {
      rc.commit(acc);
      acc = 0.f;
    }
  }
}

__device__ __forceinline__ uint32_t wave_masks(const ScheduleDev &sc, int wave, uint32_t lane) {
  const uint32_t i = lane < (uint32_t)sc.mask_stride ? lane : (uint32_t)sc.mask_stride - 1u;
  return sc.masks[(size_t)wave * sc.mask_stride + i];
}

constexpr int kWalkEnd = -1000;

template <uint32_t SRC, int RES, class AfterChunk>
__device__ __forceinline__ void walk(const Chunk6 (&res)[RES > 0 ? RES : 1], Chunk6 &qa, rsrc_t sbase,
                                     uint32_t lane16, int nchunks, uint32_t vmask, RowCommit rc,
                                     AfterChunk after_chunk TC_WALK_ARG) {
  static_assert(RES % 2 == 0, "a mask word covers two chunks");
  auto mk = [&](int i) { return (uint32_t)__builtin_amdgcn_readlane((int)vmask, i); };
  float acc = 0.f;
#ifdef TC_PHASE_STAMPS
  wst[2] = clock64();
#endif
#pragma unroll
  for (int i = 0; i < RES / 2; ++i) {
    const uint32_t m = mk(i);
    do_chunk<SRC, 0>(res[2 * i], m, acc, rc);
    after_chunk(2 * i);
    do_chunk<SRC, 1>(res[2 * i + 1], m, acc, rc);
    after_chunk(2 * i + 1);
  }
#ifdef TC_PHASE_STAMPS
  {
    __builtin_amdgcn_s_waitcnt(0xC07F);
    const long long now = clock64();
    wst[0] += now - wst[2];
    wst[2] = now;
  }
#endif
  Chunk6 qb;
  int c = RES;
  for (; c + 2 < nchunks; c += 2) {
    const uint32_t m = mk(c >> 1);
    load_chunk(qb, sbase, lane16, c + 1);
    do_chunk<SRC, 0>(qa, m, acc, rc);
    load_chunk(qa, sbase, lane16, c + 2);
    do_chunk<SRC, 1>(qb, m, acc, rc);
    if (RES == 0) after_chunk(-1 - (c >> 1));
  }
  if (c + 1 < nchunks) {
    const uint32_t m = mk(c >> 1);
    load_chunk(qb, sbase, lane16, c + 1);
    do_chunk<SRC, 0>(qa, m, acc, rc);
    do_chunk<SRC, 1>(qb, m, acc, rc);
  } else if (c < nchunks) {
    do_chunk<SRC, 0>(qa, mk(c >> 1), acc, rc);
  }
  if (RES == 0) after_chunk(kWalkEnd);
#ifdef TC_PHASE_STAMPS
  __builtin_amdgcn_s_waitcnt(0xC07F);
  wst[1] += clock64() - wst[2];
#endif
}

template <uint32_t SRC>
__device__ __forceinline__ void chunk_pw(const Chunk6 &q, uint32_t m8, float &acc, RowCommit &rc) {
  uint32_t o[8];
  o[0] = lo16w(q.oc.x);
  o[1] = hi16w(q.oc.x);
  o[2] = lo16w(q.oc.y);
  o[3] = hi16w(q.oc.y);
  o[4] = lo16w(q.oc.z);
  o[5] = hi16w(q.oc.z);
  o[6] = lo16w(q.oc.w);
  o[7] = hi16w(q.oc.w);
  float a[8];
#pragma unroll
  for (int i = 0; i < 8; ++i) a[i] = ldsf(SRC + o[i]);
  const uint32_t w[8] = {q.wa.x, q.wa.y, q.wa.z, q.wa.w, q.wb.x, q.wb.y, q.wb.z, q.wb.w};
#pragma unroll
  for (int i = 0; i < 8; ++i) {
    acc = fmaf(a[i], __uint_as_float(w[i]), acc);
    if (__builtin_expect((m8 >> i) & 1u, 0)) {
      rc.commit(acc);
      acc = 0.f;
    }
  }
}

__device__ __forceinline__ void age_prio_on(int wave) {
  if (wave >= 12)
    __builtin_amdgcn_s_setprio(3);
  else if (wave >= 8)
    __builtin_amdgcn_s_setprio(2);
  else if (wave >= 4)
    __builtin_amdgcn_s_setprio(1);
}

__device__ __forceinline__ float tied_alpha(uint32_t pb, uint32_t fs, float ws, float F, float a_self) {
  return fmaf(ldsf(pb + (fs & 0xffffu)), F, ldsf(pb + (fs >> 16)) * (ws * a_self));
}

__device__ __forceinline__ f4 own_rows(uint32_t vrow, int j) {
  return f4{ldsf(vrow + 256u * (4 * j)), ldsf(vrow + 256u * (4 * j + 1)), ldsf(vrow + 256u * (4 * j + 2)),
            ldsf(vrow + 256u * (4 * j + 3))};
}

__device__ __forceinline__ void fold_row(int2 f, uint32_t vrow, uint32_t aACC, int Hs, int K) {
  const int k = 4 * (f.x / (4 * kThreads)) + (f.x & 3);
  const uint32_t dst = vrow + 256u * (uint32_t)k;
  const uint32_t src = aACC + 256u * (uint32_t)(K * kWaves) + 4u * (uint32_t)(f.y - Hs - 4);
  ldsf_st(dst, ldsf(dst) + ldsf(src));
}

__device__ __forceinline__ void fold_row_pw(int2 f, uint32_t vrow, uint32_t aACC, int Hs) {
  const uint32_t dst = vrow + 256u * (uint32_t)(f.x & 3);
  const uint32_t src = aACC + 256u * (uint32_t)(4 * kWaves) + 4u * (uint32_t)(f.y - Hs - 4);
  ldsf_st(dst, ldsf(dst) + ldsf(src));
}

constexpr uint32_t kPlane = 16u * kThreads;

struct AsumRow {
  uint32_t lds;
  float *g;
  __device__ __forceinline__ AsumRow(const DenParams &p, int s)
      : lds(4u * (uint32_t)p.L.off_asum), g(p.L.asum_global ? p.asum_g + (int64_t)s * asum_stride(p.T) : nullptr) {}
  __device__ __forceinline__ void st(int t, float v) const {
    if (g)
      g[t] = v;
    else
      ldsf_st(lds + 4u * (uint32_t)t, v);
  }
  __device__ __forceinline__ float ld(int t) const {
    if (g) return __uint_as_float(__builtin_amdgcn_raw_buffer_load_b32(make_rsrc(g + t, 4u), 0, 0, 0));
    return ldsf(lds + 4u * (uint32_t)t);
  }
};

}

#define TC_TIED_DISPATCH(CALL)                            \
  if (JV == kJvSmall && PV == kPvSmall) return CALL(kJvSmall, kPvSmall); \
  if (JV == kJvSmall && PV == kPvMid) return CALL(kJvSmall, kPvMid);     \
  if (JV == kJvSmall && PV == kPvLarge) return CALL(kJvSmall, kPvLarge); \
  if (JV == kJvMid && PV == kPvSmall) return CALL(kJvMid, kPvSmall);     \
  if (JV == kJvMid && PV == kPvMid) return CALL(kJvMid, kPvMid);         \
  if (JV == kJvMid && PV == kPvLarge) return CALL(kJvMid, kPvLarge);     \
  if (JV == kJvLarge && PV == kPvSmall) return CALL(kJvLarge, kPvSmall); \
  if (JV == kJvLarge && PV == kPvMid) return CALL(kJvLarge, kPvMid);     \
  if (JV == kJvLarge && PV == kPvLarge) return CALL(kJvLarge, kPvLarge);

}
```

### torchain_amd/csrc/den_tied_frames.h

```cpp
#pragma once

#include <type_traits>

#include "den_tied_device.h"

namespace tc {

__device__ __forceinline__ void block_sum2(float &v1, float &v2, uint32_t red, int wave, uint32_t lane) {
  v1 = wave_sum(v1);
  v2 = wave_sum(v2);
  if (lane == 0) {
    ldsf_st(red + 4u * (uint32_t)wave, v1);
    ldsf_st(red + 4u * (uint32_t)(kWaves + wave), v2);
  }
  __syncthreads();
  float t1 = ldsf(red + 4u * (lane & 15u)), t2 = ldsf(red + 4u * (kWaves + (lane & 15u)));
  t1 = dpp_add<0xB1>(t1);
  t2 = dpp_add<0xB1>(t2);
  t1 = dpp_add<0x4E>(t1);
  t2 = dpp_add<0x4E>(t2);
  t1 = dpp_add<0x124>(t1);
  t2 = dpp_add<0x124>(t2);
  v1 = dpp_add<0x128>(t1);
  v2 = dpp_add<0x128>(t2);
}

__device__ __forceinline__ float vload_f32(const float *ptr) {
  return __uint_as_float(__builtin_amdgcn_raw_buffer_load_b32(make_rsrc(ptr, 4u), 0, 0, 0));
}

template <bool GAMMA>
__device__ __forceinline__ float tied_fwd_state(uint32_t pb, uint32_t aGM, float inv_prev, uint32_t fsx, float wsx, float Fx, float alx,
                                                float bx, float gs, float &dpart) {
  const float pf = ldsf(pb + (fsx & 0xffffu)), ps = ldsf(pb + (fsx >> 16));
  const float sp = ps * (wsx * alx);
  const float a = fmaf(pf, Fx, sp) * inv_prev;
  if constexpr (GAMMA) {
    const float g = gs * bx, spn = sp * inv_prev;
    gamma_add_a(aGM + (fsx >> 16), g * spn);
    gamma_add_a(aGM + (fsx & 0xffffu), g * fmaxf(a - spn, 0.f));
    dpart = fmaf(a, bx, dpart);
  }
  return a;
}
template <bool PURE>
__device__ __forceinline__ float tied_bwd_state(uint32_t pb, uint32_t aGM, uint32_t fsx, float wsx, float bo, float alx, float aupx,
                                                float cpx, float ax, float inv_as, float asum_up) {
  const float ps_ws = ldsf(pb + (fsx >> 16)) * wsx;
  if constexpr (!PURE) {
    const float selfpart = ps_ws * alx * inv_as;
    const float bos = kGammaScale * bo;
    gamma_add_a(aGM + (fsx >> 16), bos * selfpart);
#ifndef TC_ABL_NOFADD
    gamma_add_a(aGM + (fsx & 0xffffu), bos * fmaxf((aupx - cpx * asum_up) - selfpart, 0.f));
#endif
  }
  return fmaf(ps_ws, bo, ax);
}

template <int JV, int PV, bool ALPHA_LDS, bool ACCUM, int RESF, int RESB, bool MITM>
struct TiedSeq {
  const DenParams &p;
  const uint32_t tid, lane;
  const int wave, s;
  const int H, P, S, T, Hs, Ps;
  const int planes, K;
  const uint32_t own16, lane16;
  static constexpr uint32_t kPB = 0u;
  static constexpr uint32_t kA0 = PV * 16u * kThreads;
  const uint32_t aACC;
  const uint32_t vrow;
  const uint32_t aGM;
  const uint32_t aAL;
  const uint32_t aRed, aAsum;
  const uint32_t tab_bytes, row_bytes;
  const rsrc_t r_pi, r_fs, r_ws;
  const float leaky;
  const int64_t hist_step;
  float *const hist;
  float *const fn;
  float *const bn;
  float *const bhist;
  const int M;

  int fnch, store_slot, bnch, bstore_slot;
  uint32_t fsec, bsec;
  uint32_t aFS, aWS;
  bool tabs_lds;
  uint32_t pb_cur, pb_next;
  rsrc_t fbase, bbase;
  float asum, inv_prev, bsum;
  float chat;
  float part, y2, part_tot;
  int ffx0, ffx1, bfx0, bfx1;
  uint32_t fmask, bmask;
  Chunk6 fres[RESF > 0 ? RESF : 1];
  Chunk6 bres[RESB > 0 ? RESB : 1];
  f4 v4[JV];
  f4 bt[JV];
  f4 areg[JV];
  f4 ycur[PV], ynext[PV];
  f4 bown[JV];
#ifdef TC_PHASE_STAMPS
  long long st_prev, st_acc[8];
#endif

  __device__ __forceinline__ TiedSeq(const DenParams &pp, int seq, int meet, int frames = 0)
      : p(pp), tid(threadIdx.x), lane(threadIdx.x & 63u), wave(__builtin_amdgcn_readfirstlane(threadIdx.x >> 6)), s(seq),
        H(pp.H), P(pp.P), S(pp.S), T(frames > 0 ? frames : pp.T), Hs(pp.L.Hs), Ps(pp.L.Ps), planes(pp.L.Hs / (4 * kThreads)), K(pp.L.Hs / kThreads),
        own16(16u * threadIdx.x), lane16(16u * (threadIdx.x & 63u)), aACC(4u * (uint32_t)pp.L.off_acc),
        vrow(4u * (uint32_t)pp.L.off_acc + 256u * (uint32_t)((pp.L.Hs / kThreads) * __builtin_amdgcn_readfirstlane(threadIdx.x >> 6)) +
             4u * (threadIdx.x & 63u)),
        aGM(4u * (uint32_t)pp.L.off_g), aAL(4u * (uint32_t)pp.L.off_al), aRed(4u * (uint32_t)pp.L.off_red),
        aAsum(4u * (uint32_t)pp.L.off_asum), tab_bytes(4u * (uint32_t)(pp.L.Hs + 4)), row_bytes(4u * (uint32_t)pp.P),
        r_pi(make_rsrc(pp.pi, 4u * (uint32_t)(pp.L.Hs + 4))), r_fs(make_rsrc(pp.tied_fs, 4u * (uint32_t)(pp.L.Hs + 4))),
        r_ws(make_rsrc(pp.tied_w, 4u * (uint32_t)(pp.L.Hs + 4))), leaky(pp.leaky), hist_step((int64_t)pp.S * pp.L.Hs),
        hist(pp.alpha_hist + (int64_t)seq * pp.L.Hs), fn(MITM ? pp.fwd_norm + (int64_t)seq * (pp.T + 2) : nullptr),
        bn(MITM ? pp.bwd_norm + (int64_t)seq * (pp.T + 1) : nullptr), bhist(MITM ? pp.beta_hist + (int64_t)seq * pp.L.Hs : nullptr),
        M(meet) {}

  __device__ __forceinline__ bool plane_on(int j) const { return j < planes; }

  __device__ __forceinline__ void stamps_reset() {
#ifdef TC_PHASE_STAMPS
    st_prev = clock64();
    for (int i = 0; i < 8; ++i) st_acc[i] = 0;
#endif
  }
  __device__ __forceinline__ void stamps_flush(int base) {
#ifdef TC_PHASE_STAMPS
    TC_STAMP(0)
    if (!MITM && blockIdx.x == 0 && lane == 0)
      for (int i = 0; i < 8; ++i) p.stamps[base + wave * 8 + i] = st_acc[i];
#endif
  }

  __device__ __forceinline__ void xent_zero_row(int t) {
    if (p.xent_zero) {
      const rsrc_t xrow = make_rsrc(p.xent_zero + ((int64_t)t * S + s) * p.xent_stride, row_bytes);
#pragma unroll
      for (int v = 0; v < PV; ++v)
        if (4 * ((int)tid + kThreads * v) < Ps) row_st(xrow, own16 + v * kPlane, p.x_vec, mk4(0.f));
    }
  }

  template <bool GAMMA>
  __device__ __forceinline__ float fwd_state(uint32_t fsx, float wsx, float Fx, float alx, float bx, float gs, float &dpart) {
    return tied_fwd_state<GAMMA>(kPB, aGM, inv_prev, fsx, wsx, Fx, alx, bx, gs, dpart);
  }
  template <bool PURE>
  __device__ __forceinline__ float bwd_state(uint32_t pb, uint32_t fsx, float wsx, float bo, float alx, float aupx, float cpx, float ax,
                                             float inv_as, float asum_up) {
    return tied_bwd_state<PURE>(pb, aGM, fsx, wsx, bo, alx, aupx, cpx, ax, inv_as, asum_up);
  }

  __device__ __forceinline__ void forward_begin() {
    f4 pi4[JV];
    part = 0.f;
#pragma unroll
    for (int j = 0; j < JV; ++j) {
      pi4[j] = plane_on(j) ? bld4(r_pi, own16, j * kPlane) : mk4(0.f);
      part += hsum(pi4[j]);
    }
    asum = block_sum_a(part, aRed, wave, lane);
#pragma unroll
    for (int j = 0; j < JV; ++j)
      if (plane_on(j)) {
        const f4 a = pi4[j] + (leaky * pi4[j]) * asum;
        lds4_st(kA0 + own16 + j * kPlane, a);
        bst4(make_rsrc(hist, 4u * Hs), own16 + j * kPlane, a);
      }
    y2 = 0.f;
    {
      const rsrc_t yrow = make_rsrc(p.y + (int64_t)s * p.y_stride, row_bytes);
#pragma unroll
      for (int v = 0; v < PV; ++v) {
        const int i0 = 4 * ((int)tid + kThreads * v);
        if (i0 < Ps) {
          const f4 yv = row_ld(yrow, own16 + v * kPlane, p.y_vec);
          y2 += hsum(yv * yv);
          lds4_st(kPB + 4u * i0, exp4(yv));
        }
      }
    }
    if (tid == 0) {
      ldsf_st(aAsum, asum);
      if (MITM) fn[0] = asum;
    }
    inv_prev = __builtin_amdgcn_rcpf(asum);

    {
    const int2 frange = p.fwd.wave_range[wave];
#ifdef TC_ABL_NOSTREAM
    fnch = RESF;
#else
    fnch = __builtin_amdgcn_readfirstlane(frange.y) / kChunk;
#endif
    fbase = make_rsrc(reinterpret_cast<const char *>(p.fwd.cells) +
                          (int64_t)(__builtin_amdgcn_readfirstlane(frange.x) / kChunk) * (3 * 64 * 16),
                      (uint32_t)(fnch + 2) * (3 * 64 * 16));
    fmask = wave_masks(p.fwd, wave, lane);
    ffx0 = p.fwd.nfix ? p.fwd.fix_begin[tid] : 0;
    ffx1 = p.fwd.nfix ? p.fwd.fix_begin[tid + 1] : 0;
    fsec = aACC + 256u * (uint32_t)(K * kWaves + p.fwd.extra_first[wave]);
#pragma unroll
    for (int i = 0; i < RESF; ++i) load_chunk(fres[i], fbase, lane16, i);
    }
    tabs_lds = (p.L.off_red - p.L.off_g) >= 2 * Hs;
    aFS = aGM;
    aWS = aGM + 4u * (uint32_t)Hs;
    if (tabs_lds) {
#pragma unroll
      for (int j = 0; j < JV; ++j)
        if (plane_on(j)) {
          *reinterpret_cast<lds_u4 *>(aFS + own16 + j * kPlane) = bld4u(r_fs, own16, j * kPlane);
          lds4_st(aWS + own16 + j * kPlane, bld4(r_ws, own16, j * kPlane));
        }
    }
    store_slot = RESF >= 4 ? wave >> 2 : RESF >= 2 ? wave >> 3 : 0;
#pragma unroll
    for (int j = 0; j < JV; ++j) v4[j] = bt[j] = mk4(0.f);
    chat = 0.f;
    part_tot = 0.f;
    stamps_reset();
  }

  static constexpr bool kHistFromPass = !MITM;

  template <bool GAMMA>
  __device__ __forceinline__ void forward_frame(int t) {
#ifdef TC_PHASE_STAMPS
    long long *const wst = st_acc + 5;
#endif
    TC_STAMP(0)
    Chunk6 q0;
    load_chunk(q0, fbase, lane16, RESF);
    __syncthreads();
    TC_STAMP(1)
    f4 yreg[PV];
    if (t < T) {
      const rsrc_t yrow = make_rsrc(p.y + ((int64_t)t * S + s) * p.y_stride, row_bytes);
#pragma unroll
      for (int v = 0; v < PV; ++v) yreg[v] = row_ld(yrow, own16 + v * kPlane, p.y_vec);
    }
    float n_t = 1.f;
    if (GAMMA && t < T) n_t = vload_f32(bn + t);
    age_prio_on(wave);
    bool stored = false;
    const RowCommit frc{aACC + 256u * (uint32_t)(K * wave), fsec, K};
    walk<kA0, RESF>(fres, q0, fbase, lane16, fnch, fmask, frc, [&](int i) {
      if (!kHistFromPass && !GAMMA && t > 1 && !stored && (RESF > 0 ? i == store_slot : (i == kWalkEnd || i == -1 - (wave >> 2)))) {
        stored = true;
        const rsrc_t hist_prev = make_rsrc(hist + (int64_t)(t - 1) * hist_step, 4u * Hs);
#ifndef TC_ABL_NOHIST
#pragma unroll
        for (int j = 0; j < JV; ++j)
          if (plane_on(j)) bst4(hist_prev, own16 + j * kPlane, lds4(kA0 + own16 + j * kPlane));
#endif
      }
    } TC_WALK_PASS);
    __builtin_amdgcn_s_setprio(0);
    TC_STAMP(2)
    for (int e = ffx0; e < ffx1; ++e) fold_row(p.fwd.fix[e], vrow, aACC, Hs, K);
    TC_STAMP(3)
    part = 0.f;
    float dpart = 0.f;
    u4 fs[JV];
    f4 ws[JV], cpi[JV];
#pragma unroll
    for (int j = 0; j < JV; ++j)
      if (plane_on(j)) {
        fs[j] = tabs_lds ? lds4u(aFS + own16 + j * kPlane) : bld4u(r_fs, own16, j * kPlane);
        ws[j] = tabs_lds ? lds4(aWS + own16 + j * kPlane) : bld4(r_ws, own16, j * kPlane);
        cpi[j] = bld4(r_pi, own16, j * kPlane);
      }
    const float gs = kGammaScale * chat;
    const rsrc_t hist_prev = make_rsrc(hist + (int64_t)(t - 1) * hist_step, t > 1 ? 4u * Hs : 0u);
#pragma unroll
    for (int j = 0; j < JV; ++j) {
      v4[j] = mk4(0.f);
      if (plane_on(j)) {
        const f4 F = own_rows(vrow, j);
        const f4 al = lds4(kA0 + own16 + j * kPlane);
#ifndef TC_ABL_NOHIST
        if (kHistFromPass && !GAMMA) bst4(hist_prev, own16 + j * kPlane, al);
#endif
        v4[j] = f4{fwd_state<GAMMA>(fs[j].x, ws[j].x, F.x, al.x, bt[j].x, gs, dpart), fwd_state<GAMMA>(fs[j].y, ws[j].y, F.y, al.y, bt[j].y, gs, dpart),
                   fwd_state<GAMMA>(fs[j].z, ws[j].z, F.z, al.z, bt[j].z, gs, dpart), fwd_state<GAMMA>(fs[j].w, ws[j].w, F.w, al.w, bt[j].w, gs, dpart)};
        part += hsum(v4[j]);
      }
    }
    f4 yp[PV];
    if (GAMMA) {
      const rsrc_t yprev = make_rsrc(p.y + ((int64_t)(t - 1) * S + s) * p.y_stride, row_bytes);
#pragma unroll
      for (int v = 0; v < PV; ++v) yp[v] = row_ld(yprev, own16 + v * kPlane, p.y_vec);
      const rsrc_t brow = make_rsrc(bhist + (int64_t)(t + 1 <= T ? t + 1 : T) * hist_step, 4u * Hs);
#pragma unroll
      for (int j = 0; j < JV; ++j) bt[j] = bld4(brow, own16, j * kPlane);
      block_sum2(part, dpart, aRed, wave, lane);
      asum = part;
    } else {
      asum = block_sum_a(part, aRed, wave, lane);
    }
    __builtin_amdgcn_sched_barrier(0);
    TC_STAMP(4)
    part_tot = 0.f;
#pragma unroll
    for (int j = 0; j < JV; ++j)
      if (plane_on(j)) {
        const f4 a = v4[j] + (leaky * cpi[j]) * asum;
        lds4_st(kA0 + own16 + j * kPlane, a);
        part_tot += hsum(a);
      }
    if (GAMMA) {
      const float c = __builtin_amdgcn_rcpf(dpart);
      const float sa = p.deriv_weight * (kGammaInvScale * (c * __builtin_amdgcn_rcpf(chat)));
      const rsrc_t drow = make_rsrc(p.deriv + ((int64_t)(t - 1) * S + s) * p.deriv_stride, row_bytes);
#pragma unroll
      for (int v = 0; v < PV; ++v) {
        const int i0 = 4 * ((int)tid + kThreads * v);
        if (i0 < Ps) {
          const u4 gu = lds4u(aGM + 4u * i0);
          lds4_st(aGM + 4u * i0, mk4(0.f));
          f4 o = sa * f4{(float)gu.x, (float)gu.y, (float)gu.z, (float)gu.w} - p.l2_scale * yp[v];
          if (ACCUM) o += row_ld(drow, own16 + v * kPlane, p.d_vec);
          row_st(drow, own16 + v * kPlane, p.d_vec, o);
        }
      }
      xent_zero_row(t - 1);
      chat = c * asum * __builtin_amdgcn_rcpf(n_t);
    }
    if (t < T) {
#pragma unroll
      for (int v = 0; v < PV; ++v) {
        const int i0 = 4 * ((int)tid + kThreads * v);
        if (i0 < Ps) {
          y2 += hsum(yreg[v] * yreg[v]);
          lds4_st(kPB + 4u * i0, exp4(yreg[v]));
        }
      }
    }
    if (tid == 0) {
      ldsf_st(aAsum + 4u * t, asum);
      if (MITM) fn[t] = asum;
    }
    inv_prev = __builtin_amdgcn_rcpf(asum);
  }

  __device__ __forceinline__ void forward_unpark() {
    tabs_lds = false;
#pragma unroll
    for (int v = 0; v < PV; ++v) {
      const int i0 = 4 * ((int)tid + kThreads * v);
      if (i0 < Ps) lds4_st(aGM + 4u * i0, mk4(0.f));
    }
  }

  __device__ __forceinline__ void forward_store_row(int t) {
    const rsrc_t hist_t = make_rsrc(hist + (int64_t)t * hist_step, 4u * Hs);
#pragma unroll
    for (int j = 0; j < JV; ++j)
      if (plane_on(j)) bst4(hist_t, own16 + j * kPlane, lds4(kA0 + own16 + j * kPlane));
  }

  __device__ __forceinline__ float forward_total(double bad) {
    const float tot = block_sum_a(part_tot, aRed + 4u * kWaves, wave, lane);
    const double y2d = (double)block_sum_a(y2, aRed + 8u * kWaves, wave, lane);
    if (tid == 0) {
      double logsum = 0.0;
      for (int t = 0; t < T; ++t) logsum += (double)__logf(ldsf(aAsum + 4u * t));
      p.seq_logprob[s] = logsum + (double)__logf(tot) + (y2d - y2d) + bad;
      p.seq_y2[s] = y2d;
    }
    return tot;
  }

  __device__ __forceinline__ void backward_store_row(int t) {
    const rsrc_t brow = make_rsrc(bhist + (int64_t)t * hist_step, 4u * Hs);
#pragma unroll
    for (int j = 0; j < JV; ++j)
      if (plane_on(j)) bst4(brow, own16 + j * kPlane, bown[j]);
  }

  template <bool PURE>
  __device__ __forceinline__ void backward_begin(float b_T) {
    part = 0.f;
#pragma unroll
    for (int j = 0; j < JV; ++j)
      if (plane_on(j)) part += hsum(leaky * bld4(r_pi, own16, j * kPlane)) * b_T;
    bsum = block_sum_a(part, aRed + 12u * kWaves, wave, lane);
    pb_cur = kPB;
    pb_next = ALPHA_LDS ? 4u * (uint32_t)p.L.off_p2 : kPB;
    {
    const int2 brange = p.bwd.wave_range[wave];
#ifdef TC_ABL_NOSTREAM
    bnch = RESB;
#else
    bnch = __builtin_amdgcn_readfirstlane(brange.y) / kChunk;
#endif
    bbase = make_rsrc(reinterpret_cast<const char *>(p.bwd.cells) +
                          (int64_t)(__builtin_amdgcn_readfirstlane(brange.x) / kChunk) * (3 * 64 * 16),
                      (uint32_t)(bnch + 2) * (3 * 64 * 16));
    bmask = wave_masks(p.bwd, wave, lane);
    bfx0 = p.bwd.nfix ? p.bwd.fix_begin[tid] : 0;
    bfx1 = p.bwd.nfix ? p.bwd.fix_begin[tid + 1] : 0;
    bsec = aACC + 256u * (uint32_t)(K * kWaves + p.bwd.extra_first[wave]);
#pragma unroll
    for (int i = 0; i < RESB; ++i) load_chunk(bres[i], bbase, lane16, i);
    }
    {
      const rsrc_t hist_up = make_rsrc(hist + (int64_t)T * hist_step, 4u * Hs);
      const rsrc_t bT = make_rsrc(bhist + (int64_t)T * hist_step, PURE ? 4u * Hs : 0u);
      const rsrc_t yrow = make_rsrc(p.y + ((int64_t)(T - 1) * S + s) * p.y_stride, row_bytes);
#pragma unroll
      for (int j = 0; j < JV; ++j) {
        bown[j] = areg[j] = mk4(0.f);
        if (plane_on(j)) {
          const int h0 = 4 * ((int)tid + kThreads * j);
          const float b = b_T + bsum;
          bown[j] = f4{h0 < H ? b : 0.f, h0 + 1 < H ? b : 0.f, h0 + 2 < H ? b : 0.f, h0 + 3 < H ? b : 0.f};
          if (PURE) bst4(bT, own16 + j * kPlane, bown[j]);
          if (!PURE && ALPHA_LDS) {
            if (kHistByDma)
              areg[j] = bld4(hist_up, own16, j * kPlane);
            else
              lds4_st(aAL + own16 + j * kPlane, bld4(hist_up, own16, j * kPlane));
          }
        }
      }
#pragma unroll
      for (int v = 0; v < PV; ++v) {
        const int i0 = 4 * ((int)tid + kThreads * v);
        ycur[v] = row_ld(yrow, own16 + v * kPlane, p.y_vec);
        if (i0 < Ps) {
          lds4_st(pb_cur + 4u * i0, exp4(ycur[v]));
          lds4_st(aGM + 4u * i0, mk4(0.f));
        }
      }
      __syncthreads();
#pragma unroll
      for (int j = 0; j < JV; ++j)
        if (plane_on(j)) {
          const u4 fs = bld4u(r_fs, own16, j * kPlane);
          lds4_st(kA0 + own16 + j * kPlane,
                  f4{bown[j].x * ldsf(pb_cur + (fs.x & 0xffffu)), bown[j].y * ldsf(pb_cur + (fs.y & 0xffffu)),
                     bown[j].z * ldsf(pb_cur + (fs.z & 0xffffu)), bown[j].w * ldsf(pb_cur + (fs.w & 0xffffu))});
        }
    }
    bstore_slot = RESB >= 4 ? wave >> 2 : RESB >= 2 ? wave >> 3 : 0;
    if (!PURE && kHistByDma) hist_dma(T - 1);
    stamps_reset();
  }

#ifdef TC_NO_HIST_DMA
  static constexpr bool kHistByDma = false;
#else
  static constexpr bool kHistByDma = !MITM && ALPHA_LDS;
#endif
#ifdef TC_ABL_NOY2
  static constexpr int kDmaBehind = 3;
#else
  static constexpr int kDmaBehind = 3 + PV;
#endif

  __device__ __forceinline__ void hist_dma(int t) {
    const rsrc_t row = make_rsrc(hist + (int64_t)(t > 0 ? t : 0) * hist_step, t >= 0 ? 4u * Hs : 0u);
#pragma unroll
    for (int j = 0; j < JV; ++j)
      if (plane_on(j)) dma4_to_lds(row, own16 + j * kPlane, aAL + 1024u * (uint32_t)wave + j * kPlane);
  }

#ifdef TC_NO_BWD_DEFER
  static constexpr bool kDeferDeriv = false;
#else
  static constexpr bool kDeferDeriv = ALPHA_LDS;
#endif

  template <bool PURE>
  __device__ __forceinline__ bool backward_frame(int t, int t_top) {
#ifdef TC_PHASE_STAMPS
    long long *const wst = st_acc + 5;
#endif
    TC_STAMP(0)
    Chunk6 q0;
    load_chunk(q0, bbase, lane16, RESB);
    __syncthreads();
    TC_STAMP(1)
    const float asum_t = PURE ? 1.f : ldsf(aAsum + 4u * t);
    const float inv_as = __builtin_amdgcn_rcpf(asum_t);
    {
      const int tn = t > 0 ? t - 1 : 0;
      const rsrc_t yrow = make_rsrc(p.y + ((int64_t)tn * S + s) * p.y_stride, row_bytes);
#pragma unroll
#ifdef TC_ABL_NOY2
      for (int v = 0; v < PV; ++v) ynext[v] = mk4(0.25f) * (float)t;
#else
      for (int v = 0; v < PV; ++v) ynext[v] = row_ld(yrow, own16 + v * kPlane, p.y_vec);
#endif
      if (!PURE && !kHistByDma) {
        const rsrc_t hist_t = make_rsrc(hist + (int64_t)t * hist_step, 4u * Hs);
#pragma unroll
#ifdef TC_ABL_NOHISTLOAD
        for (int j = 0; j < JV; ++j) areg[j] = mk4(1e-4f) * (float)(t + 1);
#else
        for (int j = 0; j < JV; ++j) areg[j] = plane_on(j) ? bld4(hist_t, own16, j * kPlane) : mk4(0.f);
#endif
      }
    }
    age_prio_on(wave);
    bool dstored = false;
    const RowCommit brc{aACC + 256u * (uint32_t)(K * wave), bsec, K};
    walk<kA0, RESB>(bres, q0, bbase, lane16, bnch, bmask, brc, [&](int i) {
#ifndef TC_ABL_NOWALKSTORE
      if ((PURE ? t < T - 1 : kDeferDeriv && t < t_top - 1) && !dstored &&
          (RESB > 0 ? i == bstore_slot : (i == kWalkEnd || i == -1 - (wave >> 2)))) {
        dstored = true;
        if (PURE) {
          const rsrc_t brow_up = make_rsrc(bhist + (int64_t)(t + 1) * hist_step, 4u * Hs);
#pragma unroll
          for (int j = 0; j < JV; ++j)
            if (plane_on(j)) bst4(brow_up, own16 + j * kPlane, bown[j]);
        } else {
          const rsrc_t drow = make_rsrc(p.deriv + ((int64_t)(t + 1) * S + s) * p.deriv_stride, row_bytes);
#pragma unroll
          for (int v = 0; v < PV; ++v)
            if (4 * ((int)tid + kThreads * v) < Ps) row_st(drow, own16 + v * kPlane, p.d_vec, lds4(pb_next + own16 + v * kPlane));
          xent_zero_row(t + 1);
        }
      }
#endif
    } TC_WALK_PASS);
    __builtin_amdgcn_s_setprio(0);
    if (ALPHA_LDS) {
#pragma unroll
      for (int v = 0; v < PV; ++v) {
        const int i0 = 4 * ((int)tid + kThreads * v);
        if (i0 < Ps) lds4_st(pb_next + 4u * i0, exp4(ynext[v]));
      }
    }
    TC_STAMP(2)
    for (int e = bfx0; e < bfx1; ++e) fold_row(p.bwd.fix[e], vrow, aACC, Hs, K);
    TC_STAMP(3)
    f4 b4[JV];
    uint32_t fpk[JV][2];
    part = 0.f;
    float part_u = 0.f, part_ab = 0.f, part_g = 0.f;
    const float asum_up = PURE ? 0.f : ldsf(aAsum + 4u * (t + 1));
    constexpr bool kAhead = RESB == 0;
    u4 fs_n = u4{0u, 0u, 0u, 0u};
    f4 ws_n = mk4(0.f), cp_n = mk4(0.f), aup_n = mk4(0.f);
    auto request = [&](int j) __attribute__((always_inline)) {
      fs_n = bld4u(r_fs, own16, j * kPlane);
      ws_n = bld4(r_ws, own16, j * kPlane);
      cp_n = bld4(r_pi, own16, j * kPlane);
      if (!PURE && !ALPHA_LDS) aup_n = bld4(make_rsrc(hist + (int64_t)(t + 1) * hist_step, 4u * Hs), own16, j * kPlane);
    };
    if (!PURE && kHistByDma) dma_wait<kDmaBehind>();
    if (kAhead) request(0);
#pragma unroll
    for (int j = 0; j < JV; ++j) {
      b4[j] = mk4(0.f);
      if (plane_on(j)) {
        if (!kAhead) request(j);
        const u4 fs = fs_n;
        const f4 ws = ws_n;
        const f4 cp = leaky * cp_n;
        const f4 aup_g = aup_n;
        if (kAhead && j + 1 < planes) request(j + 1);
        f4 a = own_rows(vrow, j);
        const f4 al = (!PURE && kHistByDma) ? lds4(aAL + own16 + j * kPlane) : areg[j];
        const f4 aup = (!PURE && kHistByDma) ? areg[j] : (!PURE && ALPHA_LDS) ? lds4(aAL + own16 + j * kPlane) : aup_g;
        if (!PURE && kHistByDma) areg[j] = al;
        a.x = bwd_state<PURE>(pb_cur, fs.x, ws.x, bown[j].x, al.x, aup.x, cp.x, a.x, inv_as, asum_up);
        a.y = bwd_state<PURE>(pb_cur, fs.y, ws.y, bown[j].y, al.y, aup.y, cp.y, a.y, inv_as, asum_up);
        a.z = bwd_state<PURE>(pb_cur, fs.z, ws.z, bown[j].z, al.z, aup.z, cp.z, a.z, inv_as, asum_up);
        a.w = bwd_state<PURE>(pb_cur, fs.w, ws.w, bown[j].w, al.w, aup.w, cp.w, a.w, inv_as, asum_up);
        b4[j] = PURE ? a : a * inv_as;
        fpk[j][0] = (fs.x & 0xffffu) | (fs.y << 16);
        fpk[j][1] = (fs.z & 0xffffu) | (fs.w << 16);
        part += hsum(cp * b4[j]);
        if (PURE) part_u += hsum(a);
        if (!PURE && t == 0) part_ab += hsum(al * b4[j]);
      }
    }
    if (!PURE && kHistByDma) {
      lds_wait_all();
      hist_dma(t - 1);
    }
    float inv_n = 1.f;
    if (PURE) {
      block_sum2(part, part_u, aRed, wave, lane);
      const float n = part_u * (1.0f / (float)H);
      inv_n = __builtin_amdgcn_rcpf(n);
      bsum = part * inv_n;
      if (tid == 0) bn[t] = __builtin_amdgcn_rcpf(inv_n);
    } else {
      bsum = block_sum_a(part, aRed, wave, lane);
    }
    TC_STAMP(4)
    if (!PURE) {
      const rsrc_t drow = make_rsrc(p.deriv + ((int64_t)t * S + s) * p.deriv_stride, row_bytes);
#pragma unroll
      for (int v = 0; v < PV; ++v) {
        const int i0 = 4 * ((int)tid + kThreads * v);
        if (i0 < Ps) {
          const u4 gu = lds4u(aGM + 4u * i0);
          lds4_st(aGM + 4u * i0, mk4(0.f));
          const f4 g = f4{(float)gu.x, (float)gu.y, (float)gu.z, (float)gu.w} * kGammaInvScale;
          if (t == 0) part_g += hsum(g);
          f4 o = p.deriv_weight * g - p.l2_scale * ycur[v];
          if (ACCUM) o += row_ld(drow, own16 + v * kPlane, p.d_vec);
#ifndef TC_ABL_NODERIV
          if (kDeferDeriv && t > 0)
            lds4_st(pb_cur + 4u * i0, o);
          else
            row_st(drow, own16 + v * kPlane, p.d_vec, o);
#else
          if (o.x == 123.456f) row_st(drow, own16 + v * kPlane, p.d_vec, o);
#endif
        }
      }
      if (!(kDeferDeriv && t > 0)) xent_zero_row(t);
      if (t == 0) {
        const float ab = block_sum_a(part_ab, aRed + 4u * kWaves, wave, lane);
        const float gsum = block_sum_a(part_g, aRed + 8u * kWaves, wave, lane);
        if (tid == 0) {
          p.seq_ab[s] = ab;
          p.seq_gsum[s] = gsum;
        }
        if (kHistByDma) dma_wait<0>();
        return true;
      }
    }
    if (!ALPHA_LDS) {
#pragma unroll
      for (int v = 0; v < PV; ++v) {
        const int i0 = 4 * ((int)tid + kThreads * v);
        if (i0 < Ps) lds4_st(kPB + 4u * i0, exp4(ynext[v]));
      }
      __syncthreads();
    }
#pragma unroll
    for (int j = 0; j < JV; ++j)
      if (plane_on(j)) {
        const f4 b = PURE ? b4[j] * inv_n + bsum : b4[j] + bsum;
        bown[j] = b;
        const f4 yv = f4{b.x * ldsf(pb_next + (fpk[j][0] & 0xffffu)), b.y * ldsf(pb_next + (fpk[j][0] >> 16)),
                         b.z * ldsf(pb_next + (fpk[j][1] & 0xffffu)), b.w * ldsf(pb_next + (fpk[j][1] >> 16))};
        if constexpr (kA0 + (JV - 1) * kPlane < 65536u)
          lds4_st_at(own16, kA0 + j * kPlane, yv);
        else
          lds4_st(kA0 + own16 + j * kPlane, yv);
#ifndef TC_ABL_NOPARK
        if (!PURE && ALPHA_LDS && !kHistByDma) lds4_st(aAL + own16 + j * kPlane, areg[j]);
#endif
      }
#pragma unroll
    for (int v = 0; v < PV; ++v) ycur[v] = ynext[v];
    const uint32_t tmp = pb_cur;
    pb_cur = pb_next;
    pb_next = tmp;
    return false;
  }
};

}
```

### torchain_amd/csrc/den_tied_kernel.hip

```cpp
#include "den_tied_frames.h"

namespace tc {

namespace {

template <int JV, int PV, bool ALPHA_LDS, bool ACCUM, bool WANT_DERIV, int RESF, int RESB, bool RAGGED = false>
__global__ __launch_bounds__(kThreads) void den_tied_kernel(const DenParams p) {
  TiedSeq<JV, PV, ALPHA_LDS, ACCUM, RESF, RESB, false> q(p, (int)blockIdx.x, 0, RAGGED ? ragged_frames(p.seq_frames(), (int)blockIdx.x, p.T) : 0);
  const int T = q.T;
  q.forward_begin();
  for (int t = 1; t <= T; ++t) q.template forward_frame<false>(t);
  q.forward_store_row(T);
  q.stamps_flush(0);
  const float tot = q.forward_total(0.0);
  if (p.fwd_norm) {
    float *const fn = p.fwd_norm + (int64_t)q.s * (T + 2);
    for (int i = (int)q.tid; i <= T; i += kThreads) fn[i] = ldsf(q.aAsum + 4u * (uint32_t)i);
    if (q.tid == 0) fn[T + 1] = tot;
  }
  if (!WANT_DERIV) return;
  q.template backward_begin<false>(__builtin_amdgcn_rcpf(tot));
  for (int t = T - 1; t > 0; --t) q.template backward_frame<false>(t, T);
  q.template backward_frame<false>(0, T);
  q.stamps_flush(128);
}

#ifndef TC_RESF
#define TC_RESF 4
#endif
#ifndef TC_RESB
#define TC_RESB 4
#endif
#ifndef TC_RES_JV3
#define TC_RES_JV3 4
#endif
#ifndef TC_RES_JV4
#define TC_RES_JV4 2
#endif
constexpr int res_fwd(int jv, int pv) { return jv > 3 ? (pv == 1 ? TC_RES_JV4 : 0) : jv == 3 ? (pv == 1 ? TC_RES_JV3 : 0) : pv == 1 ? TC_RESF : 2; }
constexpr int res_bwd(int jv, int pv) { return jv > 3 ? (pv == 1 ? TC_RES_JV4 : 0) : jv == 3 ? (pv == 1 ? TC_RES_JV3 : 0) : pv == 1 ? TC_RESB : 2; }

template <int JV, int PV, bool RAGGED>
int launch_jp(const DenParams &p, int accumulate, size_t lds_bytes, hipStream_t stream) {
  constexpr int RF = res_fwd(JV, PV), RB = res_bwd(JV, PV);
  const bool want = p.deriv != nullptr;
  const bool al = p.L.alpha_in_lds;
  void (*k)(const DenParams) = nullptr;
  if (!want)
    k = den_tied_kernel<JV, PV, true, false, false, RF, RB, RAGGED>;
  else if (accumulate)
    k = al ? den_tied_kernel<JV, PV, true, true, true, RF, RB, RAGGED> : den_tied_kernel<JV, PV, false, true, true, RF, RB, RAGGED>;
  else
    k = al ? den_tied_kernel<JV, PV, true, false, true, RF, RB, RAGGED> : den_tied_kernel<JV, PV, false, false, true, RF, RB, RAGGED>;
  TC_HIP_CHECK(allow_dynamic_lds((const void *)k, lds_bytes));
  hipLaunchKernelGGL(k, dim3(p.S), dim3(kThreads), lds_bytes, stream, p);
  TC_HIP_CHECK(hipGetLastError());
  return TC_OK;
}

}

static_assert(TC_RESF <= kTiedMinChunks && TC_RESB <= kTiedMinChunks, "the resident prefix must exist in every wave's stream");

int launch_den_tied(const DenParams &p, int accumulate, hipStream_t stream) {
  const size_t lds = (size_t)layout_lds_bytes(p.L, p.T);
  if (lds > (size_t)kLdsLimitBytes) return TC_ERR_UNSUPPORTED;
  const int JV = p.L.JV, PV = p.L.PV;
  if (p.seq_frames() && p.fwd_norm) return TC_ERR_INVALID_ARGUMENT;
#define TC_CALL(J, V) (p.seq_frames() ? launch_jp<J, V, true>(p, accumulate, lds, stream) : launch_jp<J, V, false>(p, accumulate, lds, stream))
  TC_TIED_DISPATCH(TC_CALL)
#undef TC_CALL
  return TC_ERR_UNSUPPORTED;
}

}
```

Before: 28.68 million.

## Add full-layout specialization of tied denominator kernel with vectorized plane math

Adds a FULL template specialization of the tied denominator kernel. It is used when the layout exactly fills every plane and pdf slot, there are no fix rows, and vectorized row I/O applies. In that mode the per-element bounds checks, the secondary-row commit bookkeeping, fix-row folding and xent zeroing are compiled out. Per-state forward and backward math is rewritten to operate on f4 vectors, so the compiler can emit packed ops. The cost is more kernel instantiations, and the specialized path is taken only for one exact graph size.

```diff
diff --git a/profiles/full_layout/compare_isa.py b/profiles/full_layout/compare_isa.py
--- /dev/null
+++ b/profiles/full_layout/compare_isa.py
@@ -0,0 +1,108 @@
+import collections
+import os
+import re
+import subprocess
+import sys
+
+sys.path.insert(0, os.path.join(os.path.dirname(os.path.abspath(__file__)), "..", "last_pass"))
+from compare_isa import kernels
+
+FILES = ("den_tied_kernel.s", "den_tied_mitm.s", "den_tied_split.s", "den_tied_planes.s", "den_tied_pair.s", "den_general_owner.s")
+HOT = "den_tied_kernel<2, 1, true, false, true, 4, 4, false, %s>"
+
+
+def canonical(pretty):
+    name = re.sub(r"^void ", "", pretty).replace("tc::(anonymous namespace)::", "").replace("tc::", "")
+    name = re.sub(r"\((DenParams|tc::DenParams).*$", "", name)
+    m = re.match(r"den_tied_kernel<(.*)>$", name)
+    if m:
+        args = [a.strip() for a in m.group(1).split(",")]
+        args += ["false"] * (9 - len(args))
+        name = "den_tied_kernel<%s>" % ", ".join(args)
+    return name
+
+
+def load(d):
+    ks = {}
+    for f in FILES:
+        for name, v in kernels("%s/%s" % (d, f)).items():
+            ks[(f, name)] = v
+    names = [n for _, n in ks]
+    pretty = subprocess.run(["c++filt"], input="\n".join(names), stdout=subprocess.PIPE, text=True, check=True).stdout.splitlines()
+    return {(f, canonical(p)): ks[(f, n)] for (f, n), p in zip(ks, pretty)}
+
+
+def kind(op):
+    if op.startswith("v_"):
+        return "VALU"
+    if op.startswith("ds_"):
+        return "LDS"
+    if op.startswith(("buffer_", "global_", "scratch_")):
+        return "VMEM"
+    if op.startswith(("s_cbranch", "s_branch")):
+        return "branch"
+    return "other"
+
+
+def stretch(ins):
+    at = [i for i, line in enumerate(ins) if line == "s_setprio 0"]
+    if len(at) < 3:
+        return None
+    end = next(i for i in range(at[1], len(ins)) if ins[i].startswith("s_barrier"))
+    c = collections.Counter()
+    for line in ins[at[1] + 1:end]:
+        op = line.split()[0]
+        c[kind(op)] += 1
+        if op.startswith("v_mov"):
+            c["v_mov"] += 1
+        if op.startswith("v_pk_"):
+            c["v_pk"] += 1
+        if op.startswith("v_readlane"):
+            c["v_readlane"] += 1
+    return c
+
+
+def main():
+    parent, this = load(sys.argv[1]), load(sys.argv[2])
+    same = [k for k in sorted(parent) if k in this and parent[k][0] == this[k][0]]
+    print("%d of %d kernels of the parent have the same instruction text in this build" % (len(same), len(parent)))
+    for f in FILES:
+        ks = [k for k in sorted(parent) if k[0] == f]
+        bad = [k for k in ks if k not in same]
+        print("  %-22s %3d kernels, %d differ%s" % (f, len(ks), len(bad), "".join("\n      " + k[1] for k in bad)))
+    print()
+    print("kernels this build adds: instructions, VGPRs, SGPRs, spills (SGPR / VGPR), scratch bytes, v_readlane in the whole text")
+    for k in sorted(this):
+        if k not in parent:
+            ins, st = this[k]
+            print("  %5d instructions  vgpr %3d  sgpr %3d  spill %d / %d  scratch %d  readlane %d  %s" % (
+                len(ins), st["vgpr"], st["sgpr"], st["sgpr_spill"], st["vgpr_spill"], st["scratch"],
+                sum(1 for i in ins if i.startswith("v_readlane")), k[1]))
+    print()
+    print("whole kernel, hot instantiation: VGPRs, spills (SGPR / VGPR), scratch bytes, v_readlane in the text")
+    for label, table, name in (("parent", parent, HOT % "false"), ("general", this, HOT % "false"), ("FULL", this, HOT % "true")):
+        ins, st = table[("den_tied_kernel.s", name)]
+        print("  %-8s vgpr %d  spill %d / %d  scratch %d  v_readlane %d" % (
+            label, st["vgpr"], st["sgpr_spill"], st["vgpr_spill"], st["scratch"], sum(1 for i in ins if i.startswith("v_readlane"))))
+    print()
+    print("backward per-state pass of the FULL twins (backward loop's s_setprio 0 -> the reduction's s_barrier), static counts")
+    print("(the general form's stretch is not one run of text: its guarded blocks lie out of line)")
+    for k in sorted(this):
+        if k[0] == "den_tied_kernel.s" and k[1].endswith(", true>"):
+            c = stretch(this[k][0])
+            print("  VALU %3d (v_mov %d, packed %d, v_readlane %d)  LDS %d  VMEM %d  branches %d  %s" % (
+                c["VALU"], c["v_mov"], c["v_pk"], c["v_readlane"], c["LDS"], c["VMEM"], c["branch"], k[1]))
+    static = 0
+    for f in FILES:
+        try:
+            sizes = re.findall(r"\.amdhsa_group_segment_fixed_size (\d+)", open("%s/%s" % (sys.argv[2], f)).read())
+        except FileNotFoundError:
+            continue
+        static += sum(1 for x in sizes if int(x) != 0)
+    print()
+    print("kernels of this build with static LDS: %d" % static)
+    return 0 if len(same) == len(parent) and static == 0 else 1
+
+
+if __name__ == "__main__":
+    sys.exit(main())
diff --git a/torchain_amd/csrc/chain_internal.h b/torchain_amd/csrc/chain_internal.h
--- a/torchain_amd/csrc/chain_internal.h
+++ b/torchain_amd/csrc/chain_internal.h
@@ -383,6 +383,7 @@
 int launch_den(const DenParams &p, hipStream_t stream);
 int launch_den_big(const DenParams &p, int accumulate, hipStream_t stream);
 int launch_den_tied(const DenParams &p, int accumulate, hipStream_t stream);
+bool tied_full_layout(const DenParams &p);
 int launch_den_general_owner(const DenParams &p, int accumulate, hipStream_t stream);
 int launch_den_tied_planes(const DenParams &p, int accumulate, hipStream_t stream);
 bool planes_mitm_fits(const DenParams &p);
@@ -489,14 +490,14 @@
 extern thread_local int g_last_hip_error;
 
 constexpr int kKernelGeneration = 6;
-enum DebugFlag { kDbgForceGeneral = 0, kDbgForceStreamed, kDbgNoSplit, kDbgNoPdfBanks, kDbgNoBankSearch, kDbgSchedTrace, kDbgNoPhaseSplit, kDbgNoNumOverlap, kDbgNoPair, kDbgForcePair, kDbgNoTune, kDbgNoMitm, kDbgForceMitm, kDbgSlabWide, kDbgSlabNarrow, kDbgExpPerFrame, kDbgOldArrange, kDbgNoPlanes, kDbgOldGeneral, kDbgPhantomPdf0, kDbgNoPdfSearch, kDbgNoSplitSrc, kDbgPlanesMeetAt, kDbgForceNumWindowed, kDbgForceDenBestStreamed, kDbgForceNumE2eLarge, kDbgCount };
+enum DebugFlag { kDbgForceGeneral = 0, kDbgForceStreamed, kDbgNoSplit, kDbgNoPdfBanks, kDbgNoBankSearch, kDbgSchedTrace, kDbgNoPhaseSplit, kDbgNoNumOverlap, kDbgNoPair, kDbgForcePair, kDbgNoTune, kDbgNoMitm, kDbgForceMitm, kDbgSlabWide, kDbgSlabNarrow, kDbgExpPerFrame, kDbgOldArrange, kDbgNoPlanes, kDbgOldGeneral, kDbgPhantomPdf0, kDbgNoPdfSearch, kDbgNoSplitSrc, kDbgPlanesMeetAt, kDbgForceNumWindowed, kDbgForceDenBestStreamed, kDbgForceNumE2eLarge, kDbgNoFullLayout, kDbgCount };
 bool debug_flag(DebugFlag f);
 int debug_value(DebugFlag f);
 
 int pool_acquire(int device, size_t bytes, PoolSlot **out);
 void pool_release(int device, PoolSlot *slot);
 int64_t pool_counter(int which);
-enum LaunchCounter { kCntDen = 0, kCntDenBackward, kCntNum, kCntNumBackward, kCntLayout, kCntDenAsumGlobal, kCntNumE2eStaged, kCntNumWindowed, kCntChannelLast, kCntRagged, kCntRaggedTwoCu, kCntBestPath, kCntDenBestPath, kCntDenBestPathStreamed, kCntXentLogSoftmax, kCntNumE2eLarge, kCntCount };
+enum LaunchCounter { kCntDen = 0, kCntDenBackward, kCntNum, kCntNumBackward, kCntLayout, kCntDenAsumGlobal, kCntNumE2eStaged, kCntNumWindowed, kCntChannelLast, kCntRagged, kCntRaggedTwoCu, kCntBestPath, kCntDenBestPath, kCntDenBestPathStreamed, kCntXentLogSoftmax, kCntNumE2eLarge, kCntTiedFullLayout, kCntCount };
 void count_launch(LaunchCounter c);
 int supervision_mark_use(tc_supervision *sup, int device, hipStream_t stream);
 int stage_e2e_locked(tc_supervision *sup, int device);
diff --git a/torchain_amd/csrc/den_graph.cpp b/torchain_amd/csrc/den_graph.cpp
--- a/torchain_amd/csrc/den_graph.cpp
+++ b/torchain_amd/csrc/den_graph.cpp
@@ -377,7 +377,7 @@
 int tc_debug_set(const char *key, int value) {
   static const char *const names[kDbgCount] = {"force_general", "force_streamed", "no_split", "no_pdf_banks",
                                                "no_bank_search", "sched_trace", "no_phase_split", "no_num_overlap", "no_pair",
-                                               "force_pair", "no_tune", "no_mitm", "force_mitm", "slab_wide", "slab_narrow", "exp_per_frame", "old_arrange", "no_planes", "old_general", "phantom_pdf0", "no_pdf_search", "no_split_source", "planes_meet_at", "force_num_windowed", "force_den_best_path_streamed", "force_num_e2e_large"};
+                                               "force_pair", "no_tune", "no_mitm", "force_mitm", "slab_wide", "slab_narrow", "exp_per_frame", "old_arrange", "no_planes", "old_general", "phantom_pdf0", "no_pdf_search", "no_split_source", "planes_meet_at", "force_num_windowed", "force_den_best_path_streamed", "force_num_e2e_large", "no_full_layout"};
   if (!key) return TC_ERR_INVALID_ARGUMENT;
   for (int i = 0; i < kDbgCount; ++i)
     if (!strcmp(key, names[i])) {
@@ -415,7 +415,7 @@
   if (key && !strcmp(key, "pool_device_allocs")) return pool_counter(0);
   if (key && !strcmp(key, "pool_reuses")) return pool_counter(1);
   static const char *const names[kCntCount] = {"den_launches", "den_backward_launches", "num_launches", "num_backward_launches", "layout_launches",
-                                              "den_long_utterance_launches", "num_e2e_staged_launches", "num_windowed_launches", "channel_last_steps", "ragged_steps", "ragged_two_cu_launches", "best_path_launches", "den_best_path_launches", "den_best_path_streamed_launches", "xent_log_softmax_launches", "num_e2e_large_launches"};
+                                              "den_long_utterance_launches", "num_e2e_staged_launches", "num_windowed_launches", "channel_last_steps", "ragged_steps", "ragged_two_cu_launches", "best_path_launches", "den_best_path_launches", "den_best_path_streamed_launches", "xent_log_softmax_launches", "num_e2e_large_launches", "tied_full_layout_launches"};
   for (int i = 0; key && i < kCntCount; ++i)
     if (!strcmp(key, names[i])) return g_launches[i].load(std::memory_order_relaxed);
   return -1;
diff --git a/torchain_amd/csrc/den_tied_device.h b/torchain_amd/csrc/den_tied_device.h
--- a/torchain_amd/csrc/den_tied_device.h
+++ b/torchain_amd/csrc/den_tied_device.h
@@ -146,19 +146,25 @@
   return r;
 }
 
-struct RowCommit {
+template <bool SEC>
+struct RowCommitT {
   uint32_t row;
   uint32_t sec_row;
   int left;
   __device__ __forceinline__ void commit(float v) {
     asm volatile("s_mov_b32 m0, %1\n\ts_nop 0\n\tds_write_addtid_b32 %0" : : "v"(v), "s"(row) : "memory", "m0");
-    --left;
-    row = left == 0 ? sec_row : row + 256u;
+    if constexpr (SEC) {
+      --left;
+      row = left == 0 ? sec_row : row + 256u;
+    } else {
+      row += 256u;
+    }
   }
 };
-
-template <uint32_t SRC, int HALF>
-__device__ __forceinline__ void do_chunk(const Chunk6 &q, uint32_t m, float &acc, RowCommit &rc) {
+typedef RowCommitT<true> RowCommit;
+
+template <uint32_t SRC, int HALF, class RC>
+__device__ __forceinline__ void do_chunk(const Chunk6 &q, uint32_t m, float &acc, RC &rc) {
   uint32_t o[8];
   o[0] = lo16(q.oc.x);
   o[1] = hi16(q.oc.x);
@@ -196,9 +202,9 @@
 
 constexpr int kWalkEnd = -1000;
 
-template <uint32_t SRC, int RES, class AfterChunk>
+template <uint32_t SRC, int RES, class RC, class AfterChunk>
 __device__ __forceinline__ void walk(const Chunk6 (&res)[RES > 0 ? RES : 1], Chunk6 &qa, rsrc_t sbase,
-                                     uint32_t lane16, int nchunks, uint32_t vmask, RowCommit rc,
+                                     uint32_t lane16, int nchunks, uint32_t vmask, RC rc,
                                      AfterChunk after_chunk TC_WALK_ARG) {
   static_assert(RES % 2 == 0, "a mask word covers two chunks");
   auto mk = [&](int i) { return (uint32_t)__builtin_amdgcn_readlane((int)vmask, i); };
diff --git a/torchain_amd/csrc/den_tied_frames.h b/torchain_amd/csrc/den_tied_frames.h
--- a/torchain_amd/csrc/den_tied_frames.h
+++ b/torchain_amd/csrc/den_tied_frames.h
@@ -29,13 +29,41 @@
   return __uint_as_float(__builtin_amdgcn_raw_buffer_load_b32(make_rsrc(ptr, 4u), 0, 0, 0));
 }
 
-template <bool GAMMA>
-__device__ __forceinline__ float tied_fwd_state(uint32_t pb, uint32_t aGM, float inv_prev, uint32_t fsx, float wsx, float Fx, float alx,
-                                                float bx, float gs, float &dpart) {
-  const float pf = ldsf(pb + (fsx & 0xffffu)), ps = ldsf(pb + (fsx >> 16));
-  const float sp = ps * (wsx * alx);
-  const float a = fmaf(pf, Fx, sp) * inv_prev;
+__device__ __forceinline__ float vfma(float a, float b, float c) { return fmaf(a, b, c); }
+__device__ __forceinline__ f4 vfma(f4 a, f4 b, f4 c) { return __builtin_elementwise_fma(a, b, c); }
+__device__ __forceinline__ float vmax0(float a) { return fmaxf(a, 0.f); }
+__device__ __forceinline__ f4 vmax0(f4 a) { return f4{fmaxf(a.x, 0.f), fmaxf(a.y, 0.f), fmaxf(a.z, 0.f), fmaxf(a.w, 0.f)}; }
+struct LdsAt4 {
+  uint32_t base;
+  u4 off;
+};
+__device__ __forceinline__ uint32_t lds_at(uint32_t base, uint32_t off) { return base + off; }
+__device__ __forceinline__ LdsAt4 lds_at(uint32_t base, u4 off) { return LdsAt4{base, off}; }
+__device__ __forceinline__ float lds_gather(uint32_t a) { return ldsf(a); }
+__device__ __forceinline__ f4 lds_gather(LdsAt4 a) {
+  return f4{ldsf(a.base + a.off.x), ldsf(a.base + a.off.y), ldsf(a.base + a.off.z), ldsf(a.base + a.off.w)};
+}
+__device__ __forceinline__ void gamma_add_v(uint32_t a, float v) { gamma_add_a(a, v); }
+__device__ __forceinline__ void gamma_add_v(LdsAt4 a, f4 v) {
+  gamma_add_a(a.base + a.off.x, v.x);
+  gamma_add_a(a.base + a.off.y, v.y);
+  gamma_add_a(a.base + a.off.z, v.z);
+  gamma_add_a(a.base + a.off.w, v.w);
+}
+
+template <class V, class U>
+__device__ __forceinline__ V tied_fwd_sum(uint32_t pb, U fsx, V wsx, V Fx, V alx, V &sp) {
+  const V pf = lds_gather(lds_at(pb, fsx & 0xffffu)), ps = lds_gather(lds_at(pb, fsx >> 16));
+  sp = ps * (wsx * alx);
+  return vfma(pf, Fx, sp);
+}
+template <bool GAMMA, class V, class U>
+__device__ __forceinline__ V tied_fwd_state(uint32_t pb, uint32_t aGM, float inv_prev, U fsx, V wsx, V Fx, V alx, V bx, float gs,
+                                            float &dpart) {
+  V sp;
+  const V a = tied_fwd_sum(pb, fsx, wsx, Fx, alx, sp) * inv_prev;
   if constexpr (GAMMA) {
+    static_assert(std::is_same<V, float>::value, "the frames with gamma run the one-state form");
     const float g = gs * bx, spn = sp * inv_prev;
     gamma_add_a(aGM + (fsx >> 16), g * spn);
     gamma_add_a(aGM + (fsx & 0xffffu), g * fmaxf(a - spn, 0.f));
@@ -43,23 +71,28 @@
   }
   return a;
 }
-template <bool PURE>
-__device__ __forceinline__ float tied_bwd_state(uint32_t pb, uint32_t aGM, uint32_t fsx, float wsx, float bo, float alx, float aupx,
-                                                float cpx, float ax, float inv_as, float asum_up) {
-  const float ps_ws = ldsf(pb + (fsx >> 16)) * wsx;
+template <bool PURE, class V, class U>
+__device__ __forceinline__ V tied_bwd_state(uint32_t pb, uint32_t aGM, U fsx, V wsx, V bo, V alx, V aupx, V cpx, V ax, float inv_as,
+                                            float asum_up) {
+  const V ps_ws = lds_gather(lds_at(pb, fsx >> 16)) * wsx;
   if constexpr (!PURE) {
-    const float selfpart = ps_ws * alx * inv_as;
-    const float bos = kGammaScale * bo;
-    gamma_add_a(aGM + (fsx >> 16), bos * selfpart);
+    const V sa = ps_ws * alx;
+    const V selfpart = sa * inv_as;
+    const V bos = kGammaScale * bo;
+    gamma_add_v(lds_at(aGM, fsx >> 16), bos * selfpart);
 #ifndef TC_ABL_NOFADD
-    gamma_add_a(aGM + (fsx & 0xffffu), bos * fmaxf((aupx - cpx * asum_up) - selfpart, 0.f));
-#endif
-  }
-  return fmaf(ps_ws, bo, ax);
+    if constexpr (std::is_same<V, float>::value)
+      gamma_add_v(lds_at(aGM, fsx & 0xffffu), bos * vmax0((aupx - cpx * asum_up) - selfpart));
+    else
+      gamma_add_v(lds_at(aGM, fsx & 0xffffu), bos * vmax0(vfma((V)-inv_as, sa, vfma((V)-asum_up, cpx, aupx))));
+#endif
+  }
+  return vfma(ps_ws, bo, ax);
 }
 
-template <int JV, int PV, bool ALPHA_LDS, bool ACCUM, int RESF, int RESB, bool MITM>
+template <int JV, int PV, bool ALPHA_LDS, bool ACCUM, int RESF, int RESB, bool MITM, bool FULL = false>
 struct TiedSeq {
+  static_assert(!(FULL && MITM), "the two-workgroup roles run the general form");
   const DenParams &p;
   const uint32_t tid, lane;
   const int wave, s;
@@ -119,7 +152,12 @@
         bn(MITM ? pp.bwd_norm + (int64_t)seq * (pp.T + 1) : nullptr), bhist(MITM ? pp.beta_hist + (int64_t)seq * pp.L.Hs : nullptr),
         M(meet) {}
 
-  __device__ __forceinline__ bool plane_on(int j) const { return j < planes; }
+  __device__ __forceinline__ bool plane_on(int j) const { return FULL || j < planes; }
+  __device__ __forceinline__ bool pdf_on(int i0) const { return FULL || i0 < Ps; }
+  __device__ __forceinline__ int yvec() const { return FULL ? 1 : p.y_vec; }
+  __device__ __forceinline__ int dvec() const { return FULL ? 1 : p.d_vec; }
+  __device__ __forceinline__ bool tabs_parked() const { return FULL || tabs_lds; }
+  typedef RowCommitT<!FULL> Rows;
 
   __device__ __forceinline__ void stamps_reset() {
 #ifdef TC_PHASE_STAMPS
@@ -136,23 +174,23 @@
   }
 
   __device__ __forceinline__ void xent_zero_row(int t) {
-    if (p.xent_zero) {
+    if (!FULL && p.xent_zero) {
       const rsrc_t xrow = make_rsrc(p.xent_zero + ((int64_t)t * S + s) * p.xent_stride, row_bytes);
 #pragma unroll
       for (int v = 0; v < PV; ++v)
-        if (4 * ((int)tid + kThreads * v) < Ps) row_st(xrow, own16 + v * kPlane, p.x_vec, mk4(0.f));
-    }
-  }
-
-  template <bool GAMMA>
-  __device__ __forceinline__ float fwd_state(uint32_t fsx, float wsx, float Fx, float alx, float bx, float gs, float &dpart) {
+        if (pdf_on(4 * ((int)tid + kThreads * v))) row_st(xrow, own16 + v * kPlane, p.x_vec, mk4(0.f));
+    }
+  }
+
+  template <bool GAMMA, class V, class U>
+  __device__ __forceinline__ V fwd_state(U fsx, V wsx, V Fx, V alx, V bx, float gs, float &dpart) {
     return tied_fwd_state<GAMMA>(kPB, aGM, inv_prev, fsx, wsx, Fx, alx, bx, gs, dpart);
   }
-  template <bool PURE>
-  __device__ __forceinline__ float bwd_state(uint32_t pb, uint32_t fsx, float wsx, float bo, float alx, float aupx, float cpx, float ax,
-                                             float inv_as, float asum_up) {
+  template <bool PURE, class V, class U>
+  __device__ __forceinline__ V bwd_state(uint32_t pb, U fsx, V wsx, V bo, V alx, V aupx, V cpx, V ax, float inv_as, float asum_up) {
     return tied_bwd_state<PURE>(pb, aGM, fsx, wsx, bo, alx, aupx, cpx, ax, inv_as, asum_up);
   }
+  static constexpr bool kPlaneMath = FULL;
 
   __device__ __forceinline__ void forward_begin() {
     f4 pi4[JV];
@@ -162,11 +200,15 @@
       pi4[j] = plane_on(j) ? bld4(r_pi, own16, j * kPlane) : mk4(0.f);
       part += hsum(pi4[j]);
     }
-    asum = block_sum_a(part, aRed, wave, lane);
+    float asum_v = 0.f;
+    if constexpr (FULL)
+      asum = asum_v = block_sum_a(part, aRed, wave, lane);
+    else
+      asum = block_sum_a(part, aRed, wave, lane);
 #pragma unroll
     for (int j = 0; j < JV; ++j)
       if (plane_on(j)) {
-        const f4 a = pi4[j] + (leaky * pi4[j]) * asum;
+        const f4 a = pi4[j] + (leaky * pi4[j]) * (FULL ? asum_v : asum);
         lds4_st(kA0 + own16 + j * kPlane, a);
         bst4(make_rsrc(hist, 4u * Hs), own16 + j * kPlane, a);
       }
@@ -176,8 +218,8 @@
 #pragma unroll
       for (int v = 0; v < PV; ++v) {
         const int i0 = 4 * ((int)tid + kThreads * v);
-        if (i0 < Ps) {
-          const f4 yv = row_ld(yrow, own16 + v * kPlane, p.y_vec);
+        if (pdf_on(i0)) {
+          const f4 yv = row_ld(yrow, own16 + v * kPlane, yvec());
           y2 += hsum(yv * yv);
           lds4_st(kPB + 4u * i0, exp4(yv));
         }
@@ -209,7 +251,7 @@
     tabs_lds = (p.L.off_red - p.L.off_g) >= 2 * Hs;
     aFS = aGM;
     aWS = aGM + 4u * (uint32_t)Hs;
-    if (tabs_lds) {
+    if (tabs_parked()) {
 #pragma unroll
       for (int j = 0; j < JV; ++j)
         if (plane_on(j)) {
@@ -241,13 +283,13 @@
     if (t < T) {
       const rsrc_t yrow = make_rsrc(p.y + ((int64_t)t * S + s) * p.y_stride, row_bytes);
 #pragma unroll
-      for (int v = 0; v < PV; ++v) yreg[v] = row_ld(yrow, own16 + v * kPlane, p.y_vec);
+      for (int v = 0; v < PV; ++v) yreg[v] = row_ld(yrow, own16 + v * kPlane, yvec());
     }
     float n_t = 1.f;
     if (GAMMA && t < T) n_t = vload_f32(bn + t);
     age_prio_on(wave);
     bool stored = false;
-    const RowCommit frc{aACC + 256u * (uint32_t)(K * wave), fsec, K};
+    const Rows frc{aACC + 256u * (uint32_t)(K * wave), fsec, K};
     walk<kA0, RESF>(fres, q0, fbase, lane16, fnch, fmask, frc, [&](int i) {
       if (!kHistFromPass && !GAMMA && t > 1 && !stored && (RESF > 0 ? i == store_slot : (i == kWalkEnd || i == -1 - (wave >> 2)))) {
         stored = true;
@@ -261,7 +303,8 @@
     } TC_WALK_PASS);
     __builtin_amdgcn_s_setprio(0);
     TC_STAMP(2)
-    for (int e = ffx0; e < ffx1; ++e) fold_row(p.fwd.fix[e], vrow, aACC, Hs, K);
+    if constexpr (!FULL)
+      for (int e = ffx0; e < ffx1; ++e) fold_row(p.fwd.fix[e], vrow, aACC, Hs, K);
     TC_STAMP(3)
     part = 0.f;
     float dpart = 0.f;
@@ -270,8 +313,8 @@
 #pragma unroll
     for (int j = 0; j < JV; ++j)
       if (plane_on(j)) {
-        fs[j] = tabs_lds ? lds4u(aFS + own16 + j * kPlane) : bld4u(r_fs, own16, j * kPlane);
-        ws[j] = tabs_lds ? lds4(aWS + own16 + j * kPlane) : bld4(r_ws, own16, j * kPlane);
+        fs[j] = tabs_parked() ? lds4u(aFS + own16 + j * kPlane) : bld4u(r_fs, own16, j * kPlane);
+        ws[j] = tabs_parked() ? lds4(aWS + own16 + j * kPlane) : bld4(r_ws, own16, j * kPlane);
         cpi[j] = bld4(r_pi, own16, j * kPlane);
       }
     const float gs = kGammaScale * chat;
@@ -285,16 +328,22 @@
 #ifndef TC_ABL_NOHIST
         if (kHistFromPass && !GAMMA) bst4(hist_prev, own16 + j * kPlane, al);
 #endif
-        v4[j] = f4{fwd_state<GAMMA>(fs[j].x, ws[j].x, F.x, al.x, bt[j].x, gs, dpart), fwd_state<GAMMA>(fs[j].y, ws[j].y, F.y, al.y, bt[j].y, gs, dpart),
-                   fwd_state<GAMMA>(fs[j].z, ws[j].z, F.z, al.z, bt[j].z, gs, dpart), fwd_state<GAMMA>(fs[j].w, ws[j].w, F.w, al.w, bt[j].w, gs, dpart)};
-        part += hsum(v4[j]);
+        if constexpr (kPlaneMath && !GAMMA) {
+          f4 sp;
+          const f4 f = tied_fwd_sum(kPB, fs[j], ws[j], F, al, sp);
+          v4[j] = f * inv_prev;
+          part += fmaf(f.x, inv_prev, v4[j].y) + fmaf(f.z, inv_prev, v4[j].w);
+        } else
+          v4[j] = f4{fwd_state<GAMMA>(fs[j].x, ws[j].x, F.x, al.x, bt[j].x, gs, dpart), fwd_state<GAMMA>(fs[j].y, ws[j].y, F.y, al.y, bt[j].y, gs, dpart),
+                     fwd_state<GAMMA>(fs[j].z, ws[j].z, F.z, al.z, bt[j].z, gs, dpart), fwd_state<GAMMA>(fs[j].w, ws[j].w, F.w, al.w, bt[j].w, gs, dpart)};
+        if constexpr (!(kPlaneMath && !GAMMA)) part += hsum(v4[j]);
       }
     }
     f4 yp[PV];
     if (GAMMA) {
       const rsrc_t yprev = make_rsrc(p.y + ((int64_t)(t - 1) * S + s) * p.y_stride, row_bytes);
 #pragma unroll
-      for (int v = 0; v < PV; ++v) yp[v] = row_ld(yprev, own16 + v * kPlane, p.y_vec);
+      for (int v = 0; v < PV; ++v) yp[v] = row_ld(yprev, own16 + v * kPlane, yvec());
       const rsrc_t brow = make_rsrc(bhist + (int64_t)(t + 1 <= T ? t + 1 : T) * hist_step, 4u * Hs);
 #pragma unroll
       for (int j = 0; j < JV; ++j) bt[j] = bld4(brow, own16, j * kPlane);
@@ -303,13 +352,15 @@
     } else {
       asum = block_sum_a(part, aRed, wave, lane);
     }
+    float asum_v = 0.f;
+    if constexpr (FULL) asum_v = asum;
     __builtin_amdgcn_sched_barrier(0);
     TC_STAMP(4)
     part_tot = 0.f;
 #pragma unroll
     for (int j = 0; j < JV; ++j)
       if (plane_on(j)) {
-        const f4 a = v4[j] + (leaky * cpi[j]) * asum;
+        const f4 a = v4[j] + (leaky * cpi[j]) * (FULL ? asum_v : asum);
         lds4_st(kA0 + own16 + j * kPlane, a);
         part_tot += hsum(a);
       }
@@ -320,12 +371,12 @@
 #pragma unroll
       for (int v = 0; v < PV; ++v) {
         const int i0 = 4 * ((int)tid + kThreads * v);
-        if (i0 < Ps) {
+        if (pdf_on(i0)) {
           const u4 gu = lds4u(aGM + 4u * i0);
           lds4_st(aGM + 4u * i0, mk4(0.f));
           f4 o = sa * f4{(float)gu.x, (float)gu.y, (float)gu.z, (float)gu.w} - p.l2_scale * yp[v];
-          if (ACCUM) o += row_ld(drow, own16 + v * kPlane, p.d_vec);
-          row_st(drow, own16 + v * kPlane, p.d_vec, o);
+          if (ACCUM) o += row_ld(drow, own16 + v * kPlane, dvec());
+          row_st(drow, own16 + v * kPlane, dvec(), o);
         }
       }
       xent_zero_row(t - 1);
@@ -335,7 +386,7 @@
 #pragma unroll
       for (int v = 0; v < PV; ++v) {
         const int i0 = 4 * ((int)tid + kThreads * v);
-        if (i0 < Ps) {
+        if (pdf_on(i0)) {
           y2 += hsum(yreg[v] * yreg[v]);
           lds4_st(kPB + 4u * i0, exp4(yreg[v]));
         }
@@ -353,7 +404,7 @@
 #pragma unroll
     for (int v = 0; v < PV; ++v) {
       const int i0 = 4 * ((int)tid + kThreads * v);
-      if (i0 < Ps) lds4_st(aGM + 4u * i0, mk4(0.f));
+      if (pdf_on(i0)) lds4_st(aGM + 4u * i0, mk4(0.f));
     }
   }
 
@@ -432,8 +483,8 @@
 #pragma unroll
       for (int v = 0; v < PV; ++v) {
         const int i0 = 4 * ((int)tid + kThreads * v);
-        ycur[v] = row_ld(yrow, own16 + v * kPlane, p.y_vec);
-        if (i0 < Ps) {
+        ycur[v] = row_ld(yrow, own16 + v * kPlane, yvec());
+        if (pdf_on(i0)) {
           lds4_st(pb_cur + 4u * i0, exp4(ycur[v]));
           lds4_st(aGM + 4u * i0, mk4(0.f));
         }
@@ -496,7 +547,7 @@
 #ifdef TC_ABL_NOY2
       for (int v = 0; v < PV; ++v) ynext[v] = mk4(0.25f) * (float)t;
 #else
-      for (int v = 0; v < PV; ++v) ynext[v] = row_ld(yrow, own16 + v * kPlane, p.y_vec);
+      for (int v = 0; v < PV; ++v) ynext[v] = row_ld(yrow, own16 + v * kPlane, yvec());
 #endif
       if (!PURE && !kHistByDma) {
         const rsrc_t hist_t = make_rsrc(hist + (int64_t)t * hist_step, 4u * Hs);
@@ -510,7 +561,7 @@
     }
     age_prio_on(wave);
     bool dstored = false;
-    const RowCommit brc{aACC + 256u * (uint32_t)(K * wave), bsec, K};
+    const Rows brc{aACC + 256u * (uint32_t)(K * wave), bsec, K};
     walk<kA0, RESB>(bres, q0, bbase, lane16, bnch, bmask, brc, [&](int i) {
 #ifndef TC_ABL_NOWALKSTORE
       if ((PURE ? t < T - 1 : kDeferDeriv && t < t_top - 1) && !dstored &&
@@ -525,7 +576,7 @@
           const rsrc_t drow = make_rsrc(p.deriv + ((int64_t)(t + 1) * S + s) * p.deriv_stride, row_bytes);
 #pragma unroll
           for (int v = 0; v < PV; ++v)
-            if (4 * ((int)tid + kThreads * v) < Ps) row_st(drow, own16 + v * kPlane, p.d_vec, lds4(pb_next + own16 + v * kPlane));
+            if (pdf_on(4 * ((int)tid + kThreads * v))) row_st(drow, own16 + v * kPlane, dvec(), lds4(pb_next + own16 + v * kPlane));
           xent_zero_row(t + 1);
         }
       }
@@ -536,11 +587,12 @@
 #pragma unroll
       for (int v = 0; v < PV; ++v) {
         const int i0 = 4 * ((int)tid + kThreads * v);
-        if (i0 < Ps) lds4_st(pb_next + 4u * i0, exp4(ynext[v]));
+        if (pdf_on(i0)) lds4_st(pb_next + 4u * i0, exp4(ynext[v]));
       }
     }
     TC_STAMP(2)
-    for (int e = bfx0; e < bfx1; ++e) fold_row(p.bwd.fix[e], vrow, aACC, Hs, K);
+    if constexpr (!FULL)
+      for (int e = bfx0; e < bfx1; ++e) fold_row(p.bwd.fix[e], vrow, aACC, Hs, K);
     TC_STAMP(3)
     f4 b4[JV];
     uint32_t fpk[JV][2];
@@ -572,10 +624,14 @@
         const f4 al = (!PURE && kHistByDma) ? lds4(aAL + own16 + j * kPlane) : areg[j];
         const f4 aup = (!PURE && kHistByDma) ? areg[j] : (!PURE && ALPHA_LDS) ? lds4(aAL + own16 + j * kPlane) : aup_g;
         if (!PURE && kHistByDma) areg[j] = al;
-        a.x = bwd_state<PURE>(pb_cur, fs.x, ws.x, bown[j].x, al.x, aup.x, cp.x, a.x, inv_as, asum_up);
-        a.y = bwd_state<PURE>(pb_cur, fs.y, ws.y, bown[j].y, al.y, aup.y, cp.y, a.y, inv_as, asum_up);
-        a.z = bwd_state<PURE>(pb_cur, fs.z, ws.z, bown[j].z, al.z, aup.z, cp.z, a.z, inv_as, asum_up);
-        a.w = bwd_state<PURE>(pb_cur, fs.w, ws.w, bown[j].w, al.w, aup.w, cp.w, a.w, inv_as, asum_up);
+        if constexpr (kPlaneMath) {
+          a = bwd_state<PURE>(pb_cur, fs, ws, bown[j], al, aup, cp, a, inv_as, asum_up);
+        } else {
+          a.x = bwd_state<PURE>(pb_cur, fs.x, ws.x, bown[j].x, al.x, aup.x, cp.x, a.x, inv_as, asum_up);
+          a.y = bwd_state<PURE>(pb_cur, fs.y, ws.y, bown[j].y, al.y, aup.y, cp.y, a.y, inv_as, asum_up);
+          a.z = bwd_state<PURE>(pb_cur, fs.z, ws.z, bown[j].z, al.z, aup.z, cp.z, a.z, inv_as, asum_up);
+          a.w = bwd_state<PURE>(pb_cur, fs.w, ws.w, bown[j].w, al.w, aup.w, cp.w, a.w, inv_as, asum_up);
+        }
         b4[j] = PURE ? a : a * inv_as;
         fpk[j][0] = (fs.x & 0xffffu) | (fs.y << 16);
         fpk[j][1] = (fs.z & 0xffffu) | (fs.w << 16);
@@ -604,20 +660,20 @@
 #pragma unroll
       for (int v = 0; v < PV; ++v) {
         const int i0 = 4 * ((int)tid + kThreads * v);
-        if (i0 < Ps) {
+        if (pdf_on(i0)) {
           const u4 gu = lds4u(aGM + 4u * i0);
           lds4_st(aGM + 4u * i0, mk4(0.f));
           const f4 g = f4{(float)gu.x, (float)gu.y, (float)gu.z, (float)gu.w} * kGammaInvScale;
           if (t == 0) part_g += hsum(g);
           f4 o = p.deriv_weight * g - p.l2_scale * ycur[v];
-          if (ACCUM) o += row_ld(drow, own16 + v * kPlane, p.d_vec);
+          if (ACCUM) o += row_ld(drow, own16 + v * kPlane, dvec());
 #ifndef TC_ABL_NODERIV
           if (kDeferDeriv && t > 0)
             lds4_st(pb_cur + 4u * i0, o);
           else
-            row_st(drow, own16 + v * kPlane, p.d_vec, o);
+            row_st(drow, own16 + v * kPlane, dvec(), o);
 #else
-          if (o.x == 123.456f) row_st(drow, own16 + v * kPlane, p.d_vec, o);
+          if (o.x == 123.456f) row_st(drow, own16 + v * kPlane, dvec(), o);
 #endif
         }
       }
@@ -637,7 +693,7 @@
 #pragma unroll
       for (int v = 0; v < PV; ++v) {
         const int i0 = 4 * ((int)tid + kThreads * v);
-        if (i0 < Ps) lds4_st(kPB + 4u * i0, exp4(ynext[v]));
+        if (pdf_on(i0)) lds4_st(kPB + 4u * i0, exp4(ynext[v]));
       }
       __syncthreads();
     }
diff --git a/torchain_amd/csrc/den_tied_kernel.hip b/torchain_amd/csrc/den_tied_kernel.hip
--- a/torchain_amd/csrc/den_tied_kernel.hip
+++ b/torchain_amd/csrc/den_tied_kernel.hip
@@ -4,9 +4,10 @@
 
 namespace {
 
-template <int JV, int PV, bool ALPHA_LDS, bool ACCUM, bool WANT_DERIV, int RESF, int RESB, bool RAGGED = false>
+template <int JV, int PV, bool ALPHA_LDS, bool ACCUM, bool WANT_DERIV, int RESF, int RESB, bool RAGGED = false, bool FULL = false>
 __global__ __launch_bounds__(kThreads) void den_tied_kernel(const DenParams p) {
-  TiedSeq<JV, PV, ALPHA_LDS, ACCUM, RESF, RESB, false> q(p, (int)blockIdx.x, 0, RAGGED ? ragged_frames(p.seq_frames(), (int)blockIdx.x, p.T) : 0);
+  static_assert(!(FULL && RAGGED), "ragged batches run the general form");
+  TiedSeq<JV, PV, ALPHA_LDS, ACCUM, RESF, RESB, false, FULL> q(p, (int)blockIdx.x, 0, RAGGED ? ragged_frames(p.seq_frames(), (int)blockIdx.x, p.T) : 0);
   const int T = q.T;
   q.forward_begin();
   for (int t = 1; t <= T; ++t) q.template forward_frame<false>(t);
@@ -52,6 +53,12 @@
     k = al ? den_tied_kernel<JV, PV, true, true, true, RF, RB, RAGGED> : den_tied_kernel<JV, PV, false, true, true, RF, RB, RAGGED>;
   else
     k = al ? den_tied_kernel<JV, PV, true, false, true, RF, RB, RAGGED> : den_tied_kernel<JV, PV, false, false, true, RF, RB, RAGGED>;
+  if constexpr (JV == kJvSmall && PV == kPvSmall && !RAGGED) {
+    if (tied_full_layout(p)) {
+      k = accumulate ? den_tied_kernel<JV, PV, true, true, true, RF, RB, false, true> : den_tied_kernel<JV, PV, true, false, true, RF, RB, false, true>;
+      count_launch(kCntTiedFullLayout);
+    }
+  }
   TC_HIP_CHECK(allow_dynamic_lds((const void *)k, lds_bytes));
   hipLaunchKernelGGL(k, dim3(p.S), dim3(kThreads), lds_bytes, stream, p);
   TC_HIP_CHECK(hipGetLastError());
@@ -61,6 +68,22 @@
 }
 
 static_assert(TC_RESF <= kTiedMinChunks && TC_RESB <= kTiedMinChunks, "the resident prefix must exist in every wave's stream");
+
+bool tied_full_layout(const DenParams &p) {
+#if defined(TC_PHASE_STAMPS) || defined(TC_ABL_NOATOM) || defined(TC_ABL_NODERIV) || defined(TC_ABL_NOFADD) || defined(TC_ABL_NOGAM) || \
+    defined(TC_ABL_NOGATHER) || defined(TC_ABL_NOHIST) || defined(TC_ABL_NOHISTLOAD) || defined(TC_ABL_NOPARK) ||                      \
+    defined(TC_ABL_NOSTREAM) || defined(TC_ABL_NOWALKSTORE) || defined(TC_ABL_NOY2) || defined(TC_NO_BWD_DEFER) || defined(TC_NO_HIST_DMA)
+  return false;
+#else
+  if (debug_flag(kDbgNoFullLayout)) return false;
+  if (p.L.JV != kJvSmall || p.L.PV != kPvSmall || p.L.planewise) return false;
+  if (p.L.Hs != 4 * kThreads * kJvSmall || p.L.Ps != 4 * kThreads * kPvSmall || p.P != p.L.Ps) return false;
+  if (!p.L.alpha_in_lds || p.L.off_red - p.L.off_g < 2 * p.L.Hs) return false;
+  if (!p.deriv || !p.y_vec || !p.d_vec || p.xent_zero) return false;
+  if (p.fwd.nfix != 0 || p.bwd.nfix != 0) return false;
+  return p.seq_frames() == nullptr;
+#endif
+}
 
 int launch_den_tied(const DenParams &p, int accumulate, hipStream_t stream) {
   const size_t lds = (size_t)layout_lds_bytes(p.L, p.T);
```

Result: faster. 30.38 million, median of 6 (+5.9%).
